# sag111/ContiniousEnvironment_Follower_Leader

Measured on AMD Instinct MI355X. Metric: env-steps/sec at 65,536 parallel envs; 1/2/4/8 MI355X scaling, higher is better.
Workload: dtype f64

## Files before the change

continiousenvironment_follower_leader_amd/_lib.py:

```python
import ctypes as C
import os
import subprocess

from . import abi

_PKG = os.path.dirname(os.path.abspath(__file__))
_ROOT = os.path.dirname(_PKG)
SO_PATH = os.path.join(_PKG, "libftl_hip.so")
SOURCES = [os.path.join(_PKG, "csrc", "ftl_abi.hip"), os.path.join(_PKG, "csrc", "ftl_device.hpp"),
           os.path.join(_PKG, "csrc", "ftl_frames_group.hpp"), os.path.join(_PKG, "csrc", "ftl_aux.hpp"), os.path.join(_PKG, "csrc", "ftl_gazebo.hpp"), os.path.join(_ROOT, "include", "ftl_gazebo.h"), os.path.join(_PKG, "csrc", "ftl_scenario.cpp"),
           os.path.join(_PKG, "csrc", "ftl_scenario_dev.hpp"),
           os.path.join(_PKG, "csrc", "ftl_crmath.hpp"),
           os.path.join(_PKG, "csrc", "ftl_render.hpp"),
           os.path.join(_PKG, "csrc", "ftl_snapshot.hpp"),
           os.path.join(_PKG, "csrc", "ftl_queue.hpp"),
           os.path.join(_PKG, "csrc", "ftl_sampler.hpp"),
           os.path.join(_ROOT, "include", "ftl.h")]
UNITS = [os.path.join(_PKG, "csrc", "ftl_abi.hip"), os.path.join(_PKG, "csrc", "ftl_scenario.cpp")]
HIPCC = os.environ.get("HIPCC", "/opt/rocm/bin/hipcc")
HIPCC_FLAGS = ["--offload-arch=gfx950", "-O3", "-ffp-contract=off", "-fPIC", "-shared", "-std=c++17"]

_LIB = None


def build(force=False, verbose=False):
    stale = (not os.path.exists(SO_PATH)) or any(os.path.getmtime(s) > os.path.getmtime(SO_PATH) for s in SOURCES)
    if force or stale:
        cmd = [HIPCC] + HIPCC_FLAGS + ["-pthread", "-o", SO_PATH] + UNITS
        if verbose:
            print(" ".join(cmd))
        subprocess.check_call(cmd, cwd=os.path.join(_PKG, "csrc"))
    return SO_PATH


class FtlError(RuntimeError):
    pass


def load():
    global _LIB
    if _LIB is not None:
        return _LIB
    so_path = os.environ.get("FTL_LIB", SO_PATH)
    if not os.path.exists(so_path):
        raise FtlError("libftl_hip.so is not built (run `python -c 'import __graft_entry__ as g; g.build()'`); "
                       "there is no CPU fallback")
    import torch
    lib = C.CDLL(so_path)
    vp, i32, u32 = C.c_void_p, C.c_int32, C.c_uint32
    lib.ftl_last_error.restype = C.c_char_p
    lib.ftl_create.argtypes = [C.POINTER(abi.Config), i32, i32, C.POINTER(vp)]
    lib.ftl_create.restype = C.c_int
    lib.ftl_destroy.argtypes = [vp]
    lib.ftl_destroy.restype = None
    lib.ftl_lasers_len.argtypes = [vp]
    lib.ftl_lasers_len.restype = i32
    lib.ftl_get_config.argtypes = [vp, C.POINTER(abi.Config)]
    lib.ftl_state_bytes.argtypes = [vp]
    lib.ftl_state_bytes.restype = C.c_size_t
    lib.ftl_bind_state.argtypes = [vp, vp, C.c_size_t]
    lib.ftl_state_field.argtypes = [vp, C.c_char_p, C.POINTER(C.c_size_t), C.POINTER(C.c_size_t), C.POINTER(i32), C.POINTER(C.c_size_t)]
    lib.ftl_load_scenarios.argtypes = [vp, C.POINTER(abi.Scenarios)]
    lib.ftl_set_reset_window.argtypes = [vp, i32, i32, i32]
    lib.ftl_tune.argtypes = [vp, i32, i32]
    lib.ftl_reset.argtypes = [vp, vp, vp, C.POINTER(abi.Outputs), vp]
    lib.ftl_step.argtypes = [vp, vp, C.POINTER(abi.Outputs), u32, vp]
    lib.ftl_step_encoded.argtypes = [vp, vp, i32, C.POINTER(abi.Outputs), u32, vp]
    lib.ftl_step_final.argtypes = [vp, vp, i32, C.POINTER(abi.Outputs), C.POINTER(abi.FinalOutputs), u32, vp]
    lib.ftl_kernel_timing.argtypes = [vp, i32]
    lib.ftl_kernel_times.argtypes = [vp, C.POINTER(C.c_double * 4), C.POINTER(i32)]
    lib.ftl_episode_metrics.argtypes = [vp, vp, vp, u32, vp]
    lib.ftl_episode_metrics.restype = C.c_int
    lib.ftl_generate_scenarios.argtypes = [C.POINTER(abi.Config), C.POINTER(abi.ScenParams), vp, i32, i32,
                                           C.POINTER(abi.Scenarios), vp]
    lib.ftl_generate_scenarios.restype = C.c_int
    lib.ftl_sizeof_scen_params.restype = C.c_size_t
    lib.ftl_generate_scenarios_device_workspace.argtypes = [C.POINTER(abi.Config), C.POINTER(abi.ScenParams), i32, C.POINTER(C.c_size_t)]
    lib.ftl_generate_scenarios_device_workspace.restype = C.c_int
    lib.ftl_generate_scenarios_device.argtypes = [C.POINTER(abi.Config), C.POINTER(abi.ScenParams), vp, i32, C.POINTER(abi.Scenarios), vp,
                                                  vp, C.c_size_t, vp]
    lib.ftl_generate_scenarios_device.restype = C.c_int
    lib.ftl_sizeof_render_params.restype = C.c_size_t
    lib.ftl_render_workspace.argtypes = [vp, i32, C.POINTER(C.c_size_t)]
    lib.ftl_render_workspace.restype = C.c_int
    lib.ftl_render.argtypes = [vp, vp, i32, C.POINTER(abi.RenderParams), vp, C.c_size_t, vp, vp]
    lib.ftl_render.restype = C.c_int
    lib.ftl_env_bytes.argtypes = [vp]
    lib.ftl_env_bytes.restype = C.c_size_t
    lib.ftl_env_layout_id.argtypes = [vp]
    lib.ftl_env_layout_id.restype = C.c_uint64
    lib.ftl_pack_envs.argtypes = [vp, vp, i32, vp, vp]
    lib.ftl_pack_envs.restype = C.c_int
    lib.ftl_unpack_envs.argtypes = [vp, vp, vp, i32, u32, vp]
    lib.ftl_unpack_envs.restype = C.c_int
    lib.ftl_sizeof_episode_record.restype = C.c_size_t
    lib.ftl_sizeof_episode_queue.restype = C.c_size_t
    lib.ftl_set_episode_queue.argtypes = [vp, C.POINTER(abi.EpisodeQueueC)]
    lib.ftl_set_episode_queue.restype = C.c_int
    lib.ftl_queue_start.argtypes = [vp, C.POINTER(abi.Outputs), vp]
    lib.ftl_queue_start.restype = C.c_int
    lib.ftl_sizeof_scenario_sampler.restype = C.c_size_t
    lib.ftl_set_scenario_sampler.argtypes = [vp, C.POINTER(abi.ScenarioSamplerC)]
    lib.ftl_set_scenario_sampler.restype = C.c_int
    lib.ftl_sampler_refresh.argtypes = [vp, vp]
    lib.ftl_sampler_refresh.restype = C.c_int
    lib.ftl_sampler_start.argtypes = [vp, C.POINTER(abi.Outputs), vp]
    lib.ftl_sampler_start.restype = C.c_int
    lib.ftl_gz_create.argtypes = [vp, i32, i32, C.POINTER(vp)]
    lib.ftl_gz_destroy.argtypes = [vp]
    lib.ftl_gz_destroy.restype = None
    lib.ftl_gz_state_bytes.argtypes = [vp]
    lib.ftl_gz_state_bytes.restype = C.c_size_t
    lib.ftl_gz_bind_state.argtypes = [vp, vp, C.c_size_t]
    lib.ftl_gz_lasers_len.argtypes = [vp]
    lib.ftl_gz_lasers_len.restype = i32
    lib.ftl_gz_reset.argtypes = [vp, vp, vp]
    lib.ftl_gz_step.argtypes = [vp, vp, vp, vp, vp, vp, vp, vp, vp]
    lib.ftl_gz_state_field.argtypes = [vp, C.c_char_p, C.POINTER(C.c_size_t), C.POINTER(C.c_size_t), C.POINTER(i32)]
    for n in ("ftl_sizeof_config", "ftl_sizeof_scenarios", "ftl_sizeof_outputs", "ftl_sizeof_final_outputs"):
        getattr(lib, n).restype = C.c_size_t
    _LIB = lib
    return lib


EXPORTS = ("ftl_create", "ftl_destroy", "ftl_lasers_len", "ftl_get_config", "ftl_state_bytes", "ftl_bind_state",
           "ftl_state_field", "ftl_load_scenarios", "ftl_set_reset_window", "ftl_tune", "ftl_reset", "ftl_step", "ftl_step_encoded", "ftl_step_final", "ftl_last_error", "ftl_generate_scenarios",
           "ftl_generate_scenarios_device_workspace", "ftl_generate_scenarios_device",
           "ftl_episode_metrics", "ftl_kernel_timing", "ftl_kernel_times",
           "ftl_sizeof_render_params", "ftl_render_workspace", "ftl_render",
           "ftl_env_bytes", "ftl_env_layout_id", "ftl_pack_envs", "ftl_unpack_envs",
           "ftl_sizeof_episode_record", "ftl_sizeof_episode_queue", "ftl_set_episode_queue", "ftl_queue_start",
           "ftl_sizeof_scenario_sampler", "ftl_set_scenario_sampler", "ftl_sampler_refresh", "ftl_sampler_start",
           "ftl_gz_create", "ftl_gz_destroy", "ftl_gz_state_bytes", "ftl_gz_bind_state", "ftl_gz_lasers_len", "ftl_gz_reset", "ftl_gz_step",
           "ftl_gz_state_field")


def check(rc, lib=None):
    if rc != 0:
        lib = lib or load()
        msg = lib.ftl_last_error().decode("utf-8", "replace")
        if rc == abi.FTL_E_INVALID:
            raise ValueError(msg)
        if rc == abi.FTL_E_UNSUPPORTED:
            raise NotImplementedError(msg)
        raise FtlError("ftl error %d: %s" % (rc, msg))
```

continiousenvironment_follower_leader_amd/abi.py:

```python
import ctypes as C

FTL_ABI_VERSION = 4
FTL_MAX_BEARS = 6
FTL_MAX_LASERS = 4
FTL_MAX_AUX = 8
AUX_LIDAR, AUX_TRACK_VECTOR, AUX_TRACK_RADAR = 1, 2, 3
FTL_MAX_REGIME = 16
FTL_OBS_NUM = 10

FTL_OK = 0
FTL_E_INVALID, FTL_E_UNSUPPORTED, FTL_E_DEVICE, FTL_E_STATE = -1, -2, -3, -4

MISSION = ("in_progress", "fail", "success", "finished_by_time")
AGENT = ("moving", "crash", "low_reward", "too_far_from_leader", "finished")
LEADER = ("moving", "crash", "finished")

FTL_ERR_TRAJ_OVERFLOW, FTL_ERR_CORR_OVERFLOW, FTL_ERR_EMPTY_CORRIDOR, FTL_ERR_TRACKER_SEED, FTL_ERR_HIST1_OVERFLOW = 1, 2, 4, 8, 16
FTL_ERR_LIDAR_OVERFLOW = 32
FTL_ERR_BAD_ACTION = 64
FTL_ERR_BAD_STREAM = 128
FTL_ACTION_BOX2, FTL_ACTION_DISCRETE, FTL_ACTION_TURN = 0, 1, 2
FTL_STEP_AUTO_RESET = 1
FTL_STEP_NEXT_RESET = 4
FTL_STEP_QUEUE_RESET = 8
FTL_STEP_SAMPLE_RESET = 16
FTL_EPISODE_DONE_AT_RESET = 1
FTL_N_SCEN_STATS = 10
(SS_EPISODES, SS_FRAMES_SUM, SS_SUCCESS, SS_CRASH, SS_LOW_REWARD, SS_TOO_FAR, SS_TIMEOUT, SS_RETURN_Q16, SS_DONE_AT_RESET,
 SS_LAST_CALL) = range(10)
SS_NAMES = ("episodes", "frames_sum", "success", "crash", "low_reward", "too_far", "timeout", "return_q16", "done_at_reset", "last_call")
FTL_N_METRICS = 8
FTL_METRICS_CLEAR = 1
(M_EPISODES, M_RETURN_SUM, M_FRAMES_SUM, M_SUCCESS, M_CRASH, M_LOW_REWARD, M_TOO_FAR, M_TIMEOUT) = range(8)

(EI_SCEN, EI_TARGET_ID, EI_LEADER_FINISHED, EI_DONE, EI_CRASH, EI_IN_BOX, EI_ON_TRACE, EI_TOO_CLOSE,
 EI_STEP_COUNT, EI_FINISH_TIMER, EI_TRAJ_LEN, EI_TRK_COUNTER, EI_CORR_LO, EI_CORR_HI, EI_SEED_END,
 EI_SNAP_COUNT, EI_DYN_INDEX0, EI_DYN_INDEX1, EI_DYN_INDEX2, EI_DYN_INDEX3, EI_DYN_INDEX4, EI_DYN_INDEX5, EI_ERROR, EI_EPISODES,
 EI_GREEN_COUNT, EI_GREEN_LEN, EI_SCAN_OK, EI_SNAP_HEAD, EI_HINT, EI_GREEN_TINY, EI_RESETS, EI_ACC_CONSUMED,
 EI_HINT_X, EI_HINT_Y, EI_CLR_GREEN, EI_CLR_ALL, EI_FPS, EI_HW0_LO, EI_HW0_HI, EI_HIST1_LEN, EI_ERROR_STICKY, EI_STREAM, EI_COUNT) = range(43)
FTL_ENV_SLOT_STATS, FTL_ENV_OWN_STREAM = 1, 2
ED_ACC_PENALTY, ED_OVERALL_REWARD, ED_SPARE0, ED_SPARE1, ED_BEAR_POINTS = range(5)
ED_GREEN_W = ED_BEAR_POINTS + 2 * FTL_MAX_BEARS
ED_CUR_MULT, ED_CUR_ACC, ED_CUM_SPEED = ED_GREEN_W + 1, ED_GREEN_W + 2, ED_GREEN_W + 3
ED_COUNT = ED_CUM_SPEED + 1
RD_DIRECTION, RD_SPEED, RD_ROT_SPEED, RD_DES_SPEED, RD_DES_ROT_SPEED, RD_COUNT = range(6)
RI_X, RI_Y, RI_W, RI_H, RI_ROT_DIR, RI_DES_ROT_DIR, RI_SPARE0, RI_SPARE1, RI_COUNT = range(9)


def rand_frames(rng_seed, env_id, resets, step_count, lo, hi):
    v = lo + int(uniform01(rng_seed, env_id, resets, step_count | (1 << 40)) * (hi - lo))
    return v if v < hi else hi - 1


def rand_range(rng_seed, env_id, resets, frame, bear, k, start, stop):
    n = (stop - start + 9) // 10
    v = int(uniform01(rng_seed, env_id, resets, frame | (1 << 41) | (bear << 44) | (k << 48)) * n)
    return start + 10 * (v if v < n else n - 1)


class RobotParams(C.Structure):
    _fields_ = [("min_speed", C.c_double), ("max_speed", C.c_double), ("max_rotation_speed", C.c_double),
                ("max_speed_change", C.c_double), ("max_rotation_speed_change", C.c_double),
                ("img_w", C.c_int32), ("img_h", C.c_int32), ("_pad", C.c_int32 * 2)]


class LaserCfg(C.Structure):
    _fields_ = [("count", C.c_int32), ("react_corridor", C.c_int32), ("react_green", C.c_int32),
                ("react_obstacles", C.c_int32), ("history", C.c_int32), ("after_tracker", C.c_int32),
                ("out_offset", C.c_int32), ("pad_sectors", C.c_int32), ("lenient", C.c_int32), ("in_policy_obs", C.c_int32),
                ("length", C.c_double), ("angle_offset", C.c_double),
                ("explicit_angles", C.c_int32), ("compas", C.c_int32), ("ray_angles", C.c_double * 8)]


class AuxCfg(C.Structure):
    _fields_ = [("kind", C.c_int32), ("after_tracker", C.c_int32), ("out_offset", C.c_int32), ("out_len", C.c_int32),
                ("n_angles", C.c_int32), ("points_number", C.c_int32), ("return_all_points", C.c_int32),
                ("return_only_distances", C.c_int32), ("range_px", C.c_double), ("in_range_px", C.c_double),
                ("angle_step", C.c_double), ("border_angle", C.c_int32), ("seq_len", C.c_int32),
                ("detectable", C.c_int32), ("radar_sectors", C.c_int32)]


class Config(C.Structure):
    _fields_ = [("abi_version", C.c_int32), ("width", C.c_int32), ("height", C.c_int32),
                ("frames_per_step", C.c_int32), ("max_steps", C.c_int32), ("warm_start", C.c_int32),
                ("trajectory_saving_period", C.c_int32), ("n_static", C.c_int32), ("n_bears", C.c_int32),
                ("move_bear_v4", C.c_int32), ("ignore_follower_collisions", C.c_int32),
                ("aggregate_reward", C.c_int32), ("has_low_reward", C.c_int32),
                ("has_max_distance_coef", C.c_int32), ("has_tracker", C.c_int32),
                ("tracker_saving_period", C.c_int32), ("tracker_start_behind", C.c_int32),
                ("n_lasers", C.c_int32), ("traj_cap", C.c_int32), ("corr_cap", C.c_int32),
                ("route_cap", C.c_int32), ("init_traj_cap", C.c_int32), ("hist1_cap", C.c_int32), ("trk1_eat_close_points", C.c_int32),
                ("low_reward", C.c_double), ("max_distance_coef", C.c_double),
                ("min_distance", C.c_double), ("max_distance", C.c_double), ("max_dev", C.c_double),
                ("leader_pos_epsilon", C.c_double), ("corridor_length", C.c_double),
                ("corridor_width", C.c_double),
                ("reward_in_box", C.c_double), ("reward_on_track", C.c_double), ("reward_in_dev", C.c_double),
                ("not_on_track_penalty", C.c_double), ("crash_penalty", C.c_double),
                ("too_close_penalty", C.c_double), ("leader_movement_reward", C.c_double),
                ("leader", RobotParams), ("follower", RobotParams), ("bear", RobotParams),
                ("lasers", LaserCfg * FTL_MAX_LASERS),
                ("n_speed_regime", C.c_int32), ("n_acc_regime", C.c_int32),
                ("speed_key", C.c_int32 * FTL_MAX_REGIME), ("speed_is_range", C.c_int32 * FTL_MAX_REGIME),
                ("acc_key", C.c_int32 * FTL_MAX_REGIME), ("env_id_base", C.c_int32),
                ("rand_fps_lo", C.c_int32), ("rand_fps_hi", C.c_int32), ("_pad1", C.c_int32),
                ("speed_lo", C.c_double * FTL_MAX_REGIME), ("speed_hi", C.c_double * FTL_MAX_REGIME),
                ("acc_val", C.c_double * FTL_MAX_REGIME), ("rng_seed", C.c_uint64),
                ("trk1_eat_radius", C.c_double), ("n_aux", C.c_int32), ("_pad2", C.c_int32), ("aux", AuxCfg * FTL_MAX_AUX)]


_M64 = (1 << 64) - 1


def mix64(x):
    x &= _M64
    x ^= x >> 30; x = (x * 0xBF58476D1CE4E5B9) & _M64
    x ^= x >> 27; x = (x * 0x94D049BB133111EB) & _M64
    x ^= x >> 31
    return x


def uniform01(rng_seed, env_id, resets, frame):
    key = mix64(rng_seed + 0x9E3779B97F4A7C15 * (env_id + 1)) ^ mix64(0xD1B54A32D192ED03 * (resets + 1))
    return (mix64(key + 0x9E3779B97F4A7C15 * (frame + 1)) >> 11) * (1.0 / 9007199254740992.0)


def mulhi64(a, b):
    return ((a & _M64) * (b & _M64)) >> 64


def sample_scenario(rng_seed, stream_id, resets, cdf, base=0):
    key = mix64(rng_seed + 0x9E3779B97F4A7C15 * (stream_id + 1)) ^ mix64(0xD1B54A32D192ED03 * (resets + 1))
    x = mix64(key + 0x9E3779B97F4A7C15 * ((1 << 42) + 1))
    count = len(cdf)
    total = int(cdf[count - 1])
    if total == 0:
        return base + mulhi64(x, count)
    r = mulhi64(x, total)
    lo, hi = 0, count - 1
    while lo < hi:
        mid = lo + (hi - lo) // 2
        if int(cdf[mid]) <= r:
            lo = mid + 1
        else:
            hi = mid
    return base + lo


class Scenarios(C.Structure):
    _fields_ = [("n_scenarios", C.c_int32), ("_pad", C.c_int32),
                ("static_rects", C.c_void_p), ("robot_pos", C.c_void_p), ("robot_dir", C.c_void_p),
                ("robot_rect", C.c_void_p), ("route", C.c_void_p), ("route_len", C.c_void_p),
                ("init_traj", C.c_void_p), ("init_traj_len", C.c_void_p)]


class ScenParams(C.Structure):
    _fields_ = [("width", C.c_int32), ("height", C.c_int32), ("step_grid", C.c_int32), ("obstacle_number", C.c_int32),
                ("add_obstacles", C.c_int32), ("add_bear", C.c_int32), ("bear_number", C.c_int32), ("bear_behind", C.c_int32),
                ("multiple_end_points", C.c_int32), ("path_finding_iterations", C.c_int32),
                ("bridge_gap", C.c_int32), ("bridge_width", C.c_int32),
                ("trajectory_saving_period", C.c_int32), ("planner", C.c_int32),
                ("min_distance", C.c_double), ("max_distance", C.c_double),
                ("leader_pos_epsilon", C.c_double), ("leader_margin", C.c_double),
                ("leader_w", C.c_double), ("leader_h", C.c_double), ("leader_max_speed", C.c_double),
                ("fixed_route", C.c_void_p), ("fixed_route_len", C.c_int32), ("_pad", C.c_int32)]


SCEN_FOUND, SCEN_DONE_AT_RESET, SCEN_ROUTE_OVERFLOW, SCEN_TRAJ_OVERFLOW, SCEN_REF_RAISES = 1, 2, 4, 8, 16
SCEN_GEN_LIMIT = 32


class Outputs(C.Structure):
    _fields_ = [("obs_num", C.c_void_p), ("lasers", C.c_void_p), ("target", C.c_void_p),
                ("reward", C.c_void_p), ("done", C.c_void_p), ("status", C.c_void_p), ("policy_obs", C.c_void_p)]

FTL_TUNE_COSCHEDULED_ENVS, FTL_TUNE_REGROUP_EVERY, FTL_TUNE_TWO_STREAMS = 0, 1, 2


class FinalOutputs(C.Structure):
    _fields_ = [("obs_num", C.c_void_p), ("lasers", C.c_void_p), ("target", C.c_void_p), ("policy_obs", C.c_void_p),
                ("ended", C.c_void_p), ("restarted", C.c_void_p)]


class EpisodeRecord(C.Structure):
    _fields_ = [("state", C.c_int32), ("scenario", C.c_int32), ("env", C.c_int32), ("frames", C.c_int32), ("calls", C.c_int32),
                ("status", C.c_int32 * 3), ("errors", C.c_uint32), ("flags", C.c_uint32), ("ret", C.c_double), ("stream", C.c_int64)]


RECORD_DTYPE = [("state", "<i4"), ("scenario", "<i4"), ("env", "<i4"), ("frames", "<i4"), ("calls", "<i4"), ("status", "<i4", (3,)),
                ("errors", "<u4"), ("flags", "<u4"), ("ret", "<f8"), ("stream", "<i8")]


class EpisodeQueueC(C.Structure):
    _fields_ = [("scenario", C.c_void_p), ("stream", C.c_void_p), ("stream_base", C.c_int64), ("n", C.c_int32), ("_pad", C.c_int32),
                ("head", C.c_void_p), ("records", C.c_void_p), ("ticket", C.c_void_p)]


class ScenarioSamplerC(C.Structure):
    _fields_ = [("weight", C.c_void_p), ("cdf", C.c_void_p), ("base", C.c_int32), ("count", C.c_int32), ("table", C.c_void_p)]


RENDER_PATH, RENDER_BOX, RENDER_OBJECTS, RENDER_RECTS, RENDER_SENSORS, RENDER_TARGET = 1, 2, 4, 8, 16, 32
RENDER_ALL = 63


class RenderParams(C.Structure):
    _fields_ = [("width", C.c_int32), ("height", C.c_int32), ("scale", C.c_float), ("origin_x", C.c_float), ("origin_y", C.c_float),
                ("layers", C.c_uint32), ("_pad", C.c_int32)]
```

continiousenvironment_follower_leader_amd/csrc/ftl_abi.hip:

```cpp
#include <hip/hip_runtime.h>

#include <cstdio>
#include <cstring>
#include <new>
#include <string>
#include <vector>

#include <cstdlib>
#include <cmath>

#include "ftl_device.hpp"
#include "ftl_frames_group.hpp"
#include "ftl_aux.hpp"

namespace {

thread_local std::string g_err;

int fail(int code, const std::string& msg) { g_err = msg; return code; }

struct Field { const char* name; size_t offset, per_env; int dtype; size_t stride; };
constexpr int FTL_N_FIELDS = 15;

}

struct FtlQueueState;
struct FtlSamplerState;

struct ftl_handle {
    FtlDevParams P;
    FtlDevParams* dP;
    bool dirty;
    int device;
    size_t state_bytes;
    Field fields[FTL_N_FIELDS];
    void* mt_mem;
    bool timing;
    std::vector<hipEvent_t> tev;
    size_t tev_used;
    bool bound, have_scen;
    bool regroup;
    void* rg_mem;
    int* rg_tot;
    unsigned rg_parity, rg_launches, rg_every;
    bool rg_env, rg_every_env, split_env;
    int G;
    int co_envs, cus;
    bool g_env;
    int rg_slots, rg_epw;
    hipStream_t side; hipEvent_t ev_fork, ev_join; bool split;
    int win_base, win_count, win_stride;
    size_t lds_pad;
    float* last_lasers;
    FtlQueueState* queue;
    FtlSamplerState* sampler;
};

static void ftl_queue_destroy(ftl_handle* h);
static int ftl_queue_attached(const ftl_handle* h);
static int ftl_queue_finish_step(ftl_handle* h, const FtlCall& step, const ftl_outputs* out, const ftl_final_outputs* fin, void* stream);
static void ftl_sampler_destroy(ftl_handle* h);
static int ftl_sampler_attached(const ftl_handle* h);
static int ftl_sampler_check_window(const ftl_handle* h);
static int ftl_sampler_finish_step(ftl_handle* h, const FtlCall& step, const ftl_outputs* out, const ftl_final_outputs* fin, void* stream);

namespace {

size_t align_up(size_t v, size_t a) { return (v + a - 1) / a * a; }

int validate(const ftl_config& c, std::string& why) {
    char buf[256];
#define REQ(cond, ...) do { if (!(cond)) { snprintf(buf, sizeof buf, __VA_ARGS__); why = buf; return FTL_E_INVALID; } } while (0)
    REQ(c.abi_version == FTL_ABI_VERSION, "abi_version %d != %d", c.abi_version, FTL_ABI_VERSION);
    REQ(c.width > 0 && c.height > 0, "bad field size");
    REQ(c.frames_per_step > 0, "frames_per_step must be positive");
    REQ(c.rand_fps_hi == 0 || (c.rand_fps_lo > 0 && c.rand_fps_lo < c.rand_fps_hi), "random_frames_per_step must be (low, high) with 0 < low < high");
    REQ(c.trajectory_saving_period > 0, "trajectory_saving_period must be positive");
    REQ(c.n_static >= 0 && c.n_static <= 4096, "n_static out of range");
    REQ(c.n_bears >= 0 && c.n_bears <= FTL_MAX_BEARS, "n_bears out of range (0..%d)", FTL_MAX_BEARS);
    REQ(c.n_lasers >= 0 && c.n_lasers <= FTL_MAX_LASERS, "n_lasers out of range");
    REQ(c.n_lasers == 0 || c.has_tracker, "ray sensors need the tracker (classes.py:280 would raise NameError)");
    REQ(c.traj_cap >= 8 && c.corr_cap >= 8 && c.corr_cap <= 512 && c.route_cap >= 2 && c.init_traj_cap >= 1, "bad capacities");
    REQ((c.corr_cap & (c.corr_cap - 1)) == 0, "corr_cap must be a power of two (the tracker rings are indexed with a mask)");
    REQ(c.init_traj_cap <= c.traj_cap, "init_traj_cap > traj_cap");
    REQ(c.traj_cap % FTL_TRAJ_BLOCK == 0, "traj_cap must be a multiple of FTL_TRAJ_BLOCK");
    if (c.has_tracker == 2) {
        REQ(c.tracker_saving_period > 0, "tracker saving_period must be positive");
        REQ(c.corridor_length > 0 && c.corridor_width > 0, "corridor_length / corridor_width must be positive");
    }
    REQ(c.n_speed_regime <= FTL_MAX_REGIME && c.n_acc_regime <= FTL_MAX_REGIME, "too many regime entries");
    REQ(c.has_tracker >= 0 && c.has_tracker <= 2, "has_tracker must be 0, 1 (v1) or 2 (v2)");
    if (c.has_tracker == 1) REQ(c.tracker_saving_period > 0 && c.hist1_cap >= 8 && c.corridor_width > 0, "bad v1 tracker parameters");
    REQ(c.n_aux >= 0 && c.n_aux <= FTL_MAX_AUX, "n_aux out of range");
    for (int j = 0; j < c.n_aux; j++) {
        const ftl_aux_cfg& a = c.aux[j];
        REQ(a.kind >= FTL_AUX_LIDAR && a.kind <= FTL_AUX_TRACK_RADAR, "aux %d: unknown sensor kind", j);
        if (a.kind == FTL_AUX_LIDAR) {
            REQ(a.n_angles > 0 && a.n_angles <= 512 && a.points_number > 0 && a.range_px > 0, "aux %d: bad lidar parameters", j);
            REQ(a.points_number <= 1024 && a.n_angles * a.points_number < 65536, "aux %d: lidar with more than 1024 points per ray or 65535 (ray, point) pairs", j);
        }
        else {
            REQ(c.has_tracker != 0, "aux %d: a leader-track detector needs a tracker (classes.py:272 would raise NameError)", j);
            REQ(a.seq_len > 0 && a.detectable >= 0 && a.detectable <= (a.kind == FTL_AUX_TRACK_RADAR ? 2 : 1), "aux %d: bad detector parameters", j);
            if (a.kind == FTL_AUX_TRACK_RADAR) REQ(a.radar_sectors > 0 && a.radar_sectors <= 4096, "aux %d: bad radar_sectors_number", j);
        }
    }
    for (int k = 0; k < c.n_lasers; k++) {
        const ftl_laser_cfg& l = c.lasers[k];
        REQ(l.count > 0 && l.count <= 1024, "laser %d: bad lasers_count", k);
        REQ(l.history > 0 && l.history <= FTL_HMAX, "laser %d: max_prev_obs must be in 1..%d", k, FTL_HMAX);
        REQ(l.react_obstacles >= 0 && l.react_obstacles <= 3, "laser %d: bad react_to_obstacles", k);
        REQ(l.length > 0, "laser %d: bad laser_length", k);
    }
#undef REQ
    return FTL_OK;
}

}

extern "C" {

const char* ftl_last_error(void) { return g_err.c_str(); }

size_t ftl_sizeof_config(void) { return sizeof(ftl_config); }
size_t ftl_sizeof_scenarios(void) { return sizeof(ftl_scenarios); }
size_t ftl_sizeof_outputs(void) { return sizeof(ftl_outputs); }
size_t ftl_sizeof_scen_params(void) { return sizeof(ftl_scen_params); }
size_t ftl_sizeof_final_outputs(void) { return sizeof(ftl_final_outputs); }

static int set_lanes(ftl_handle* h) {
    FtlDevParams& P = h->P;
    const ftl_config* cfg = &P.cfg;
    if (!h->g_env) h->G = (P.R > 4 || h->co_envs <= h->cus * 4 * 8) ? 8 : 4;
    if (P.R > 4) h->G = 8;
    const int epw = FTL_WAVE / h->G;
    h->rg_epw = epw;
    const int f_max = cfg->rand_fps_hi > 0 ? cfg->rand_fps_hi - 1 : cfg->frames_per_step;
    size_t o = align_up((size_t)epw * cfg->n_static * 16 + (size_t)epw * 4 + 32, 16);
    P.fr_rec_stride = (int)align_up((size_t)f_max, 16);
    P.fr_rec_off = (int)o; o += (size_t)P.fr_rec_stride * epw;
    P.fr_pend_off = (int)o; o += (size_t)epw * (P.fr_defer ? f_max - 1 : 1) * 16;
    P.fr_env_off = (int)o; o += (size_t)epw * 4 + 16 + (size_t)epw * 16;
    P.fr_lds = (int)o;
    h->dirty = true;
    return o > 64 * 1024 ? 1 : 0;
}

int ftl_create(const ftl_config* cfg, int32_t n_envs, int32_t device, ftl_handle** out) {
    if (!cfg || !out) return fail(FTL_E_INVALID, "null argument");
    if (n_envs <= 0) return fail(FTL_E_INVALID, "n_envs must be positive");
    if (device < 0) return fail(FTL_E_INVALID, "device < 0: this library has no CPU path");
    std::string why;
    int rc = validate(*cfg, why);
    if (rc) return fail(rc, why);
    ftl_handle* h = new (std::nothrow) ftl_handle();
    if (!h) return fail(FTL_E_DEVICE, "out of host memory");
    memset(&h->P, 0, sizeof h->P);
    h->P.cfg = *cfg;
    for (int k = 0; k < FTL_MAX_LASERS; k++) h->P.cfg.lasers[k].after_tracker = cfg->lasers[k].after_tracker ? 1 : 0;
    h->device = device;
    h->bound = false; h->have_scen = false; h->dP = nullptr; h->dirty = true;
    h->rg_mem = nullptr; h->rg_tot = nullptr; h->rg_parity = 0; h->rg_launches = 0; h->mt_mem = nullptr; h->timing = false; h->tev_used = 0;
    h->side = nullptr; h->ev_fork = nullptr; h->ev_join = nullptr; h->last_lasers = nullptr; h->queue = nullptr; h->sampler = nullptr;
    {
        const char* sp = getenv("FTL_SPLIT");
        h->split = n_envs >= 8192 && (sp ? sp[0] == '1' : cfg->rand_fps_hi > 0) && cfg->has_tracker != 1;
        h->split_env = sp != nullptr;
    }
    {
        const char* off = getenv("FTL_NO_REGROUP");
        const char* ev = getenv("FTL_REGROUP_EVERY");
        h->rg_every = (ev && atoi(ev) > 0) ? (unsigned)atoi(ev) : 4u;
        int cus = 256;
        (void)hipDeviceGetAttribute(&cus, hipDeviceAttributeMultiprocessorCount, device);
        const char* g8 = getenv("FTL_DEBUG_G8");
        h->g_env = g8 != nullptr; h->cus = cus; h->co_envs = n_envs;
        h->G = (2 + cfg->n_bears > 4 || (g8 ? g8[0] == '1' : n_envs <= cus * 4 * 8)) ? 8 : 4;
        const int epw_f = FTL_WAVE / h->G;
        const bool beyond_one_round = (n_envs + epw_f - 1) / epw_f > cus * 4 * FTL_FRAMESG_WPE;
        h->regroup = (off ? off[0] != '1' : (beyond_one_round || cfg->rand_fps_hi > 0)) && (n_envs + FTL_RG_BLOCK - 1) / FTL_RG_BLOCK <= 512;
        h->rg_env = off != nullptr; h->rg_every_env = ev && atoi(ev) > 0; h->rg_slots = cus * 4 * FTL_FRAMESG_WPE; h->rg_epw = epw_f;
    }
    FtlDevParams& P = h->P;
    P.n_envs = n_envs;
    P.R = 2 + cfg->n_bears;
    int off = 0, hmax = 1, rays = 0;
    auto width_of = [](const ftl_laser_cfg& l) { return l.count * (l.compas ? 5 : (l.pad_sectors ? 4 : 1)); };
    for (int k = 0; k < cfg->n_lasers; k++) {
        P.cfg.lasers[k].out_offset = off;
        off += cfg->lasers[k].history * width_of(cfg->lasers[k]);
        hmax = cfg->lasers[k].history > hmax ? cfg->lasers[k].history : hmax;
        rays += cfg->lasers[k].count;
    }
    for (int j = 0; j < cfg->n_aux; j++) {
        ftl_aux_cfg& a = P.cfg.aux[j];
        a.out_len = a.kind == FTL_AUX_LIDAR ? (a.return_all_points ? 1 + a.n_angles * a.points_number * (a.return_only_distances ? 1 : 2) : a.n_angles * (a.return_only_distances ? 1 : 2))
                  : a.kind == FTL_AUX_TRACK_VECTOR ? 2 * a.seq_len : a.radar_sectors;
        a.out_offset = off; off += a.out_len;
    }
    P.lasers_len = off; P.total_rays = rays; P.hmax = hmax;
    {
        const double deg2rad = 3.141592653589793 / 180.0;
        bool miss_ok = true;
        const double span = (double)(cfg->width > cfg->height ? cfg->width : cfg->height);
        const double margin = 1e-11 * (span > 2048.0 ? span / 2048.0 : 1.0);
        for (int k = 0; k < cfg->n_lasers; k++) {
            const ftl_laser_cfg& l = cfg->lasers[k];
            miss_ok = miss_ok && (float)(l.length - margin) == (float)l.length && (float)(l.length + margin) == (float)l.length;
        }
        P.miss_const = miss_ok ? 1 : 0;
        int rb[2] = {0, 0};
        for (int k = 0; k < cfg->n_lasers; k++) {
            const ftl_laser_cfg& l = cfg->lasers[k];
            FtlRaySensor& rs = P.ray_sens[k];
            const int which = l.after_tracker ? 1 : 0, ro = l.react_obstacles;
            rs.count = l.count; rs.rbase = rb[which];
            rs.reach2 = ((float)l.length + 2.0f) * ((float)l.length + 2.0f);
            rs.inv_step = (float)l.count * 0.15915494309189535f; rs.inv_count = 1.0f / (float)l.count;
            rs.off_u = (float)(l.angle_offset * deg2rad) * rs.inv_step;
            rs.slack = 0.022f + 0.01f * (float)l.count * 0.15915494f;
            rs.flags = ((ro == 1 || ro == 2) ? 1u : 0u) | ((ro == 1 || ro == 3) ? 2u : 0u) | (l.react_corridor ? 4u : 0u) | (l.react_green ? 8u : 0u)
                     | (l.explicit_angles ? 16u : 0u) | (which ? 32u : 0u) | (l.compas ? 64u : 0u);
            if (!l.compas) rb[which] += l.count;
        }
        P.inv_nrect_dyn = (65536u + (unsigned)(P.R - 1) - 1u) / (unsigned)(P.R - 1);
        int g = 0;
        for (int which = 0; which < 2; which++) {
            P.pass_base[which] = g; P.pass_lmax[which] = 0.0f;
            for (int k = 0; k < cfg->n_lasers; k++) {
                const ftl_laser_cfg& l = cfg->lasers[k];
                if ((l.after_tracker ? 1 : 0) != which || l.compas) continue;
                P.pass_lmax[which] = fmaxf(P.pass_lmax[which], (float)l.length);
                for (int i = 0; i < l.count && g < FTL_MAX_RAYS; i++, g++) {
                    const double a = l.explicit_angles ? l.ray_angles[i & 7] : l.angle_offset + i * (360.0 / (double)l.count);
                    P.ray_dir[g].c = cos(a * deg2rad); P.ray_dir[g].s = sin(a * deg2rad); P.ray_dir[g].len = l.length;
                }
            }
            P.pass_rays[which] = g - P.pass_base[which];
        }
    }
    if (rays > 1023) { delete h; return fail(FTL_E_INVALID, "more than 1023 rays per env (the candidate list of the ray kernel packs a ray index into 10 bits)"); }
    if (hmax * (P.R - 1) > FTL_WAVE) { delete h; return fail(FTL_E_INVALID, "max_prev_obs x (1 + bears) exceeds one wavefront of snapshot rects"); }
    {
        int w = 0, hcommon = 0;
        for (int k = 0; k < cfg->n_lasers; k++) {
            P.pol_off[k] = -1;
            if (!cfg->lasers[k].in_policy_obs) continue;
            P.pol_off[k] = w; w += width_of(cfg->lasers[k]);
            if (hcommon == 0) hcommon = cfg->lasers[k].history;
            else if (cfg->lasers[k].history != hcommon) hcommon = -1;
        }
        P.pol_width = w; P.pol_h = hcommon;
    }
    const size_t n = (size_t)n_envs;
    struct { const char* name; size_t per_env; int dtype; size_t esz; bool rec; } spec[FTL_N_FIELDS] = {
        {"rb_pos", (size_t)P.R * 2, 1, 4, true}, {"rb_dbl", (size_t)P.R * FTL_RD_COUNT, 2, 8, true}, {"rb_int", (size_t)P.R * FTL_RI_COUNT, 0, 4, true},
        {"env_int", FTL_EI_COUNT, 0, 4, true}, {"env_dbl", FTL_ED_COUNT, 2, 8, true}, {"traj", (size_t)cfg->traj_cap * 2, 1, 4, false},
        {"hist", (size_t)cfg->corr_cap * 2, 2, 8, false}, {"corr", (size_t)cfg->corr_cap * 4, 2, 8, false},
        {"snap_rects", (size_t)hmax * (P.R - 1) * 4, 0, 4, true}, {"snap_win", (size_t)hmax * 4, 0, 4, true},
        {"traj_bb", (size_t)(cfg->traj_cap / FTL_TRAJ_BLOCK) * 4, 1, 4, false}, {"ep_stats", FTL_N_METRICS, 2, 8, false},
        {"hist1", (size_t)(cfg->has_tracker == 1 ? cfg->hist1_cap : 0) * 2, 1, 4, false}, {"fol_cs", 2, 2, 8, true},
        {"corr32", (size_t)cfg->corr_cap * 4, 1, 4, false}};
    static const int rec_order[8] = {3 , 13 , 0 , 1 , 9 , 8 , 4 , 2 };
    size_t ro = 0;
    for (int k = 0; k < 8; k++) {
        const int i = rec_order[k];
        ro = align_up(ro, 16);
        h->fields[i] = Field{spec[i].name, ro, spec[i].per_env, spec[i].dtype, 0};
        ro += spec[i].per_env * spec[i].esz;
    }
    const size_t rec_stride = align_up(ro, 128);
    P.rec_stride = (int32_t)rec_stride;
    for (int k = 0; k < 8; k++) h->fields[rec_order[k]].stride = rec_stride;
    size_t cur = rec_stride * n;
    for (int i = 0; i < FTL_N_FIELDS; i++) {
        if (spec[i].rec) continue;
        cur = align_up(cur, 256);
        h->fields[i] = Field{spec[i].name, cur, spec[i].per_env, spec[i].dtype, spec[i].per_env * spec[i].esz};
        cur += spec[i].per_env * spec[i].esz * n;
    }
    h->state_bytes = align_up(cur, 256);
    {
        const size_t rects = (size_t)cfg->n_static + hmax + (size_t)hmax * (P.R - 2 > 0 ? P.R - 2 : 0) + 1;
        P.corr_lds_cap = cfg->corr_cap < 128 ? cfg->corr_cap : 128;
        if (const char* lc = getenv("FTL_DEBUG_CORR_LDS_CAP")) { int v = atoi(lc); if (v >= 2 && v <= cfg->corr_cap && (v & (v - 1)) == 0) P.corr_lds_cap = v; }
        P.lds_rays = (int)((size_t)P.corr_lds_cap * 16 + rects * 20 + (size_t)2 * P.corr_lds_cap * 4 + (size_t)2 * hmax * 20 + 64
                           + (size_t)rays * 16 + (size_t)rays * (hmax <= 5 ? 5 : FTL_HMAX) * 4       + (size_t)rays * 4
                           + rects * 8 + 32
                           + (size_t)FTL_PAIR_CAP * 2 + 16);
    }
    {
        const int f_max = cfg->rand_fps_hi > 0 ? cfg->rand_fps_hi - 1 : cfg->frames_per_step;
        const char* dv = getenv("FTL_DEFER");
        P.fr_defer = (cfg->rand_fps_hi == 0 && f_max >= 2 && f_max <= 16 && cfg->traj_cap <= 65535 && !(dv && dv[0] == '0')) ? 1 : 0;
        if (cfg->traj_cap > 65535 || f_max > 4095) { delete h; return fail(FTL_E_INVALID, "traj_cap above 65535 or more than 4095 frames per step"); }
        if (set_lanes(h)) { delete h; return fail(FTL_E_INVALID, "the frame kernel needs more than 64 KiB of LDS per wavefront (static rects x frames per step)"); }
    }
    auto debug_pad = [](const char* name) { const char* v = getenv(name); const int p = v ? atoi(v) : 0; return p < 0 ? 0 : (p > 48 * 1024 ? 48 * 1024 : p); };
    P.lds_rays += debug_pad("FTL_DEBUG_LDS_PAD_RAYS");
    h->lds_pad = (size_t)debug_pad("FTL_DEBUG_LDS_PAD");
    if (getenv("FTL_DEBUG_PRINT_LDS")) fprintf(stderr, "ftl: ray kernel LDS %d B per env\n", P.lds_rays);
    if (P.lds_rays > 64 * 1024) { delete h; return fail(FTL_E_INVALID, "config needs more than 64 KiB of LDS per env"); }
    if (ftl_aux_lds_bytes(*cfg) > 64 * 1024) { delete h; return fail(FTL_E_INVALID, "the compas / lidar / radar sensors of this config need more than 64 KiB of LDS per env"); }
    *out = h;
    return FTL_OK;
}

void ftl_destroy(ftl_handle* h) {
    if (!h) return;
    if (h->dP || h->rg_mem || h->side || h->mt_mem) (void)hipSetDevice(h->device);
    ftl_queue_destroy(h);
    ftl_sampler_destroy(h);
    if (h->dP) (void)hipFree(h->dP);
    if (h->mt_mem) (void)hipFree(h->mt_mem);
    for (hipEvent_t ev : h->tev) (void)hipEventDestroy(ev);
    if (h->rg_mem) (void)hipFree(h->rg_mem);
    if (h->side) { (void)hipStreamSynchronize(h->side); (void)hipStreamDestroy(h->side); }
    if (h->ev_fork) (void)hipEventDestroy(h->ev_fork);
    if (h->ev_join) (void)hipEventDestroy(h->ev_join);
    delete h;
}

int32_t ftl_lasers_len(const ftl_handle* h) { return h ? h->P.lasers_len : 0; }

int ftl_get_config(const ftl_handle* h, ftl_config* out) {
    if (!h || !out) return fail(FTL_E_INVALID, "null argument");
    *out = h->P.cfg;
    return FTL_OK;
}

size_t ftl_state_bytes(const ftl_handle* h) { return h ? h->state_bytes : 0; }

int ftl_state_field(const ftl_handle* h, const char* name, size_t* offset, size_t* per_env, int32_t* dtype, size_t* stride) {
    if (!h || !name) return fail(FTL_E_INVALID, "null argument");
    for (int i = 0; i < FTL_N_FIELDS; i++)
        if (!strcmp(h->fields[i].name, name)) {
            if (offset) *offset = h->fields[i].offset;
            if (per_env) *per_env = h->fields[i].per_env;
            if (dtype) *dtype = h->fields[i].dtype;
            if (stride) *stride = h->fields[i].stride;
            return FTL_OK;
        }
    return fail(FTL_E_INVALID, std::string("unknown state field ") + name);
}

int ftl_bind_state(ftl_handle* h, void* dev_state, size_t bytes) {
    if (!h || !dev_state) return fail(FTL_E_INVALID, "null argument");
    if (bytes < h->state_bytes) return fail(FTL_E_INVALID, "state buffer too small");
    if (((uintptr_t)dev_state) & 255) return fail(FTL_E_INVALID, "state buffer must be 256-byte aligned");
    unsigned char* b = (unsigned char*)dev_state;
    FtlDevParams& P = h->P;
    P.rb_pos = (float*)(b + h->fields[0].offset); P.rb_dbl = (double*)(b + h->fields[1].offset); P.rb_int = (int32_t*)(b + h->fields[2].offset);
    P.env_int = (int32_t*)(b + h->fields[3].offset); P.env_dbl = (double*)(b + h->fields[4].offset); P.traj = (float*)(b + h->fields[5].offset);
    P.hist = (double*)(b + h->fields[6].offset); P.corr = (double*)(b + h->fields[7].offset);
    P.snap_rects = (int32_t*)(b + h->fields[8].offset); P.snap_win = (int32_t*)(b + h->fields[9].offset);
    P.traj_bb = (float*)(b + h->fields[10].offset); P.ep_stats = (double*)(b + h->fields[11].offset);
    P.hist1 = (float*)(b + h->fields[12].offset); P.fol_cs = (double*)(b + h->fields[13].offset); P.corr32 = (float*)(b + h->fields[14].offset);
    h->bound = true; h->dirty = true;
    return FTL_OK;
}

int ftl_load_scenarios(ftl_handle* h, const ftl_scenarios* pool) {
    if (!h || !pool) return fail(FTL_E_INVALID, "null argument");
    if (pool->n_scenarios <= 0) return fail(FTL_E_INVALID, "empty scenario pool");
    if (!pool->robot_pos || !pool->robot_dir || !pool->robot_rect || !pool->route || !pool->route_len ||
        !pool->init_traj || !pool->init_traj_len || (h->P.cfg.n_static > 0 && !pool->static_rects))
        return fail(FTL_E_INVALID, "scenario pool has null arrays");
    h->P.scen = *pool;
    h->have_scen = true; h->dirty = true;
    h->win_base = 0; h->win_count = pool->n_scenarios; h->win_stride = h->P.n_envs % pool->n_scenarios;
    return FTL_OK;
}

int ftl_set_reset_window(ftl_handle* h, int32_t base, int32_t count, int32_t stride) {
    if (!h) return fail(FTL_E_INVALID, "null argument");
    if (!h->have_scen) return fail(FTL_E_STATE, "ftl_load_scenarios has not been called");
    if (base < 0 || count <= 0 || base + count > h->P.scen.n_scenarios) return fail(FTL_E_INVALID, "reset window outside the scenario pool");
    h->win_base = base; h->win_count = count; h->win_stride = (stride > 0 ? stride : h->P.n_envs) % count;
    return FTL_OK;
}

int ftl_tune(ftl_handle* h, int32_t what, int32_t value) {
    if (!h) return fail(FTL_E_INVALID, "null argument");
    switch (what) {
    case FTL_TUNE_COSCHEDULED_ENVS:
        if (value < h->P.n_envs) return fail(FTL_E_INVALID, "co-scheduled envs below this handle's own");
        h->co_envs = value;
        if (set_lanes(h)) return fail(FTL_E_INVALID, "the frame kernel needs more than 64 KiB of LDS per wavefront (static rects x frames per step)");
        if (!h->rg_env)
            h->regroup = ((value + h->rg_epw - 1) / h->rg_epw > h->rg_slots || h->P.cfg.rand_fps_hi > 0) && (h->P.n_envs + FTL_RG_BLOCK - 1) / FTL_RG_BLOCK <= 512;
        return FTL_OK;
    case FTL_TUNE_REGROUP_EVERY:
        if (value < 1) return fail(FTL_E_INVALID, "regroup interval below 1");
        if (!h->rg_every_env) h->rg_every = (unsigned)value;
        return FTL_OK;
    case FTL_TUNE_TWO_STREAMS:
        if (!h->split_env) h->split = value != 0 && h->P.n_envs >= 8192 && h->P.cfg.has_tracker != 1;
        return FTL_OK;
    }
    return fail(FTL_E_INVALID, "unknown tuning key");
}

static int sync_params(ftl_handle* h) {
    hipError_t e;
    if (!h->dP) {
        e = hipMalloc((void**)&h->dP, sizeof(FtlDevParams));
        if (e != hipSuccess) return fail(FTL_E_DEVICE, std::string("hipMalloc(params): ") + hipGetErrorString(e));
        h->dirty = true;
    }
    if (h->dirty) {
        e = hipMemcpy(h->dP, &h->P, sizeof(FtlDevParams), hipMemcpyHostToDevice);
        if (e != hipSuccess) return fail(FTL_E_DEVICE, std::string("hipMemcpy(params): ") + hipGetErrorString(e));
        h->dirty = false;
    }
    return FTL_OK;
}

static int launch(ftl_handle* h, const FtlCall& call, void* stream) {
    hipError_t e = hipSetDevice(h->device);
    if (e != hipSuccess) return fail(FTL_E_DEVICE, std::string("hipSetDevice: ") + hipGetErrorString(e));
    if (h->regroup && !h->rg_mem) {
        const size_t n = (size_t)h->P.n_envs, nb = (n + FTL_RG_BLOCK - 1) / FTL_RG_BLOCK;
        const size_t o_bh = align_up(n * 4, 256), o_rank = o_bh + align_up(nb * FTL_NKEYS * 4, 256), o_keys = o_rank + align_up(n * 2, 256), o_tot = o_keys + align_up(n, 256);
        e = hipMalloc(&h->rg_mem, o_tot + 2 * FTL_NKEYS * sizeof(int));
        if (e != hipSuccess) return fail(FTL_E_DEVICE, std::string("hipMalloc(regroup): ") + hipGetErrorString(e));
        char* b = (char*)h->rg_mem;
        h->P.perm = (int32_t*)b; h->P.bh = (int32_t*)(b + o_bh); h->P.rank = (uint16_t*)(b + o_rank); h->P.keys = (uint8_t*)(b + o_keys);
        h->rg_tot = (int*)(b + o_tot); h->rg_parity = 0;
        e = hipMemsetAsync(h->rg_tot, 0, 2 * FTL_NKEYS * sizeof(int), (hipStream_t)stream);
        if (e != hipSuccess) return fail(FTL_E_DEVICE, std::string("hipMemsetAsync(regroup): ") + hipGetErrorString(e));
        hipLaunchKernelGGL(ftl::ftl_perm_identity_kernel, dim3((unsigned)((n + 255) / 256)), dim3(256), 0, (hipStream_t)stream, h->P.perm, (int)n);
        h->dirty = true;
    }
    { int rc = sync_params(h); if (rc) return rc; }
    if (h->split && !h->side) {
        if (hipStreamCreateWithFlags(&h->side, hipStreamNonBlocking) != hipSuccess ||
            hipEventCreateWithFlags(&h->ev_fork, hipEventDisableTiming) != hipSuccess ||
            hipEventCreateWithFlags(&h->ev_join, hipEventDisableTiming) != hipSuccess)
            return fail(FTL_E_DEVICE, "cannot create the side stream / events");
    }
    hipEvent_t* tev = nullptr;
    if (h->timing && !h->split && call.mode == 0 && h->tev_used + 5 <= 5 * 512) {
        while (h->tev.size() < h->tev_used + 5) { hipEvent_t ev; if (hipEventCreate(&ev) != hipSuccess) return fail(FTL_E_DEVICE, "hipEventCreate"); h->tev.push_back(ev); }
        tev = h->tev.data() + h->tev_used; h->tev_used += 5;
    }
    const bool xr = (call.flags & (FTL_STEP_NEXT_RESET | FTL_CALL_DEFER_RESET | FTL_CALL_FINISH)) != 0 || call.ended || call.restarted;
    auto launch_range = [&](int part, int parts, hipStream_t s) {
        const int epw0 = FTL_WAVE / h->G;
        const int n_groups = (h->P.n_envs + epw0 - 1) / epw0;
        const int my_groups = (n_groups - part + parts - 1) / parts;
        FtlCall c2 = call; c2.part = part; c2.parts = parts; c2.epw = epw0;
        const int count = my_groups * epw0;
        const bool reg = h->P.cfg.n_speed_regime >= 0 || h->P.cfg.n_acc_regime >= 0 || h->P.cfg.rand_fps_hi > 0;
        const int epw = FTL_WAVE / h->G;
        size_t lds = (size_t)h->P.fr_lds + h->lds_pad;
        const dim3 grid((count + epw - 1) / epw), block(FTL_WAVE);
        if (tev) (void)hipEventRecord(tev[0], s);
        if (xr) {
            if (h->G == 4) {
                if (reg) hipLaunchKernelGGL((ftl_frames_group_kernel<4, true, true>), grid, block, lds, s, h->dP, c2);
                else hipLaunchKernelGGL((ftl_frames_group_kernel<4, false, true>), grid, block, lds, s, h->dP, c2);
            } else {
                if (reg) hipLaunchKernelGGL((ftl_frames_group_kernel<8, true, true>), grid, block, lds, s, h->dP, c2);
                else hipLaunchKernelGGL((ftl_frames_group_kernel<8, false, true>), grid, block, lds, s, h->dP, c2);
            }
        } else if (h->G == 4) {
            if (reg) hipLaunchKernelGGL((ftl_frames_group_kernel<4, true>), grid, block, lds, s, h->dP, c2);
            else hipLaunchKernelGGL((ftl_frames_group_kernel<4, false>), grid, block, lds, s, h->dP, c2);
        } else {
            if (reg) hipLaunchKernelGGL((ftl_frames_group_kernel<8, true>), grid, block, lds, s, h->dP, c2);
            else hipLaunchKernelGGL((ftl_frames_group_kernel<8, false>), grid, block, lds, s, h->dP, c2);
        }
        if (h->P.cfg.has_tracker == 1 && part == 0)
            hipLaunchKernelGGL(ftl::ftl_tracker1_kernel, dim3((unsigned)((h->P.n_envs + 255) / 256)), dim3(256), 0, s, h->dP, c2);
        if (tev) (void)hipEventRecord(tev[1], s);
        if (h->P.cfg.n_lasers > 0) {
            bool expl = false;
            for (int k = 0; k < h->P.cfg.n_lasers; k++) expl = expl || h->P.cfg.lasers[k].explicit_angles != 0 || h->P.cfg.lasers[k].pad_sectors != 0 || h->P.cfg.lasers[k].compas != 0;
            const dim3 rgrid(count);
#define FTL_LAUNCH_RAYS(HM_, EXPL_, SPLIT_) do { \
                if (capped) hipLaunchKernelGGL((ftl_rays_kernel<HM_, EXPL_, SPLIT_, true>), rgrid, block, h->P.lds_rays, s, h->dP, c2); \
                else hipLaunchKernelGGL((ftl_rays_kernel<HM_, EXPL_, SPLIT_, false>), rgrid, block, h->P.lds_rays, s, h->dP, c2); } while (0)
            const bool capped = h->P.corr_lds_cap < h->P.cfg.corr_cap;
            if (parts > 1) {
                if (!expl && h->P.hmax > 5 && h->P.hmax <= 10) FTL_LAUNCH_RAYS(10, false, true);
                else if (h->P.hmax <= 5) FTL_LAUNCH_RAYS(5, true, true);
                else FTL_LAUNCH_RAYS(FTL_HMAX, true, true);
            } else if (expl) {
                if (h->P.hmax <= 5) FTL_LAUNCH_RAYS(5, true, false);
                else FTL_LAUNCH_RAYS(FTL_HMAX, true, false);
            } else if (h->P.hmax <= 5) FTL_LAUNCH_RAYS(5, false, false);
            else if (h->P.hmax <= 8) FTL_LAUNCH_RAYS(8, false, false);
            else if (h->P.hmax <= 10) FTL_LAUNCH_RAYS(10, false, false);
            else FTL_LAUNCH_RAYS(FTL_HMAX, false, false);
#undef FTL_LAUNCH_RAYS
        }
        if (tev) (void)hipEventRecord(tev[2], s);
    };
    if (h->split) {
        (void)hipEventRecord(h->ev_fork, (hipStream_t)stream);
        (void)hipStreamWaitEvent(h->side, h->ev_fork, 0);
        launch_range(0, 2, (hipStream_t)stream);
        launch_range(1, 2, h->side);
        (void)hipEventRecord(h->ev_join, h->side);
        (void)hipStreamWaitEvent((hipStream_t)stream, h->ev_join, 0);
    } else launch_range(0, 1, (hipStream_t)stream);
    {
        bool aux = h->P.cfg.n_aux > 0;
        for (int k = 0; k < h->P.cfg.n_lasers; k++) aux = aux || h->P.cfg.lasers[k].compas != 0;
        if (aux) hipLaunchKernelGGL(ftl_aux_kernel, dim3((unsigned)h->P.n_envs), dim3(FTL_WAVE), ftl_aux_lds_bytes(h->P.cfg), (hipStream_t)stream, h->dP, call);
    }
    if (tev) (void)hipEventRecord(tev[3], (hipStream_t)stream);
    if (h->regroup && !(call.flags & FTL_CALL_FINISH) && (h->P.cfg.rand_fps_hi > 0 || call.mode == 1 || (h->rg_launches++ % h->rg_every) == 0)) {
        const unsigned nb = (unsigned)((h->P.n_envs + FTL_RG_BLOCK - 1) / FTL_RG_BLOCK);
        int* tot = h->rg_tot + (h->rg_parity & 1u) * FTL_NKEYS, *tot_next = h->rg_tot + ((h->rg_parity + 1u) & 1u) * FTL_NKEYS;
        h->rg_parity++;
        hipLaunchKernelGGL(ftl::ftl_regroup_count_kernel, dim3(nb), dim3(FTL_RG_BLOCK), 0, (hipStream_t)stream, h->dP, tot);
        hipLaunchKernelGGL(ftl::ftl_regroup_scatter_kernel, dim3(nb), dim3(FTL_RG_BLOCK), 0, (hipStream_t)stream, h->dP, (const int*)tot, tot_next);
    }
    if (tev) (void)hipEventRecord(tev[4], (hipStream_t)stream);
    e = hipGetLastError();
    if (e != hipSuccess) return fail(FTL_E_DEVICE, std::string("kernel launch: ") + hipGetErrorString(e));
    return FTL_OK;
}

static int check_out(const ftl_handle* h, const ftl_outputs* out) {
    if (!out || !out->obs_num || !out->target || !out->reward || !out->done || !out->status || (h->P.lasers_len > 0 && !out->lasers))
        return fail(FTL_E_INVALID, "output arrays missing");
    return FTL_OK;
}

int ftl_reset(ftl_handle* h, const int32_t* scen_idx, const uint8_t* mask, const ftl_outputs* out, void* stream) {
    if (!h || !scen_idx) return fail(FTL_E_INVALID, "null argument");
    if (!h->bound) return fail(FTL_E_STATE, "ftl_bind_state has not been called");
    if (!h->have_scen) return fail(FTL_E_STATE, "ftl_load_scenarios has not been called");
    int rc = check_out(h, out);
    if (rc) return rc;
    if (out->policy_obs && h->P.pol_h <= 0) return fail(FTL_E_INVALID, "policy_obs needs the same max_prev_obs on every ray sensor");
    FtlCall call; call.mode = 1; call.scen_idx = scen_idx; call.mask = mask; call.out = *out; call.action = nullptr; call.flags = 0; call.action_kind = FTL_ACTION_BOX2; call.win_base = h->win_base; call.win_count = h->win_count; call.win_stride = h->win_stride;
    call.ended = nullptr; call.restarted = nullptr;
    h->last_lasers = h->P.lasers_len > 0 ? out->lasers : nullptr;
    return launch(h, call, stream);
}

int ftl_step(ftl_handle* h, const double* action, const ftl_outputs* out, uint32_t flags, void* stream) {
    return ftl_step_encoded(h, action, FTL_ACTION_BOX2, out, flags, stream);
}

int ftl_step_encoded(ftl_handle* h, const void* action, int32_t encoding, const ftl_outputs* out, uint32_t flags, void* stream) {
    return ftl_step_final(h, action, encoding, out, nullptr, flags, stream);
}

int ftl_step_final(ftl_handle* h, const void* action, int32_t encoding, const ftl_outputs* out, const ftl_final_outputs* fin,
                   uint32_t flags, void* stream) {
    if (!h || !action) return fail(FTL_E_INVALID, "null argument");
    flags &= FTL_STEP_AUTO_RESET | FTL_STEP_NEXT_RESET | FTL_STEP_QUEUE_RESET | FTL_STEP_SAMPLE_RESET;
    if ((flags & FTL_STEP_AUTO_RESET) && (flags & FTL_STEP_NEXT_RESET)) return fail(FTL_E_INVALID, "FTL_STEP_AUTO_RESET and FTL_STEP_NEXT_RESET exclude each other");
    const bool queue = (flags & FTL_STEP_QUEUE_RESET) != 0;
    if (queue && flags != FTL_STEP_QUEUE_RESET) return fail(FTL_E_INVALID, "FTL_STEP_QUEUE_RESET excludes the other reset flags");
    const bool sample = (flags & FTL_STEP_SAMPLE_RESET) != 0;
    if (sample && flags != FTL_STEP_SAMPLE_RESET) return fail(FTL_E_INVALID, "FTL_STEP_SAMPLE_RESET excludes the other reset flags");
    if (encoding < FTL_ACTION_BOX2 || encoding > FTL_ACTION_TURN) return fail(FTL_E_INVALID, "unknown action encoding");
    if (sample && !ftl_sampler_attached(h)) return fail(FTL_E_STATE, "FTL_STEP_SAMPLE_RESET without a scenario sampler (ftl_set_scenario_sampler)");
    if (queue && !ftl_queue_attached(h)) return fail(FTL_E_STATE, "FTL_STEP_QUEUE_RESET without an episode queue (ftl_set_episode_queue)");
    if (!h->bound) return fail(FTL_E_STATE, "ftl_bind_state has not been called");
    if (!h->have_scen) return fail(FTL_E_STATE, "ftl_load_scenarios has not been called");
    int rc = check_out(h, out);
    if (rc) return rc;
    if (out->policy_obs && h->P.pol_h <= 0) return fail(FTL_E_INVALID, "policy_obs needs the same max_prev_obs on every ray sensor");
    const bool same_step = fin && (flags & (FTL_STEP_AUTO_RESET | FTL_STEP_QUEUE_RESET | FTL_STEP_SAMPLE_RESET));
    if (fin && (!fin->ended || !fin->restarted)) return fail(FTL_E_INVALID, "ftl_final_outputs: ended / restarted missing");
    if (same_step && (!fin->obs_num || !fin->target || (h->P.lasers_len > 0 && !fin->lasers)))
        return fail(FTL_E_INVALID, "ftl_final_outputs: obs_num / lasers / target missing (needed under FTL_STEP_AUTO_RESET / FTL_STEP_QUEUE_RESET / FTL_STEP_SAMPLE_RESET)");
    if (same_step && fin->policy_obs && !out->policy_obs) return fail(FTL_E_INVALID, "ftl_final_outputs.policy_obs needs ftl_outputs.policy_obs");
    FtlCall call; call.mode = 0; call.action = (const double*)action; call.action_kind = encoding; call.out = *out; call.flags = flags; call.scen_idx = nullptr; call.mask = nullptr; call.win_base = h->win_base; call.win_count = h->win_count; call.win_stride = h->win_stride;
    call.ended = fin ? fin->ended : nullptr; call.restarted = fin ? fin->restarted : nullptr;
    h->last_lasers = h->P.lasers_len > 0 ? out->lasers : nullptr;
    if (queue) {
        call.flags = 0; call.ended = nullptr; call.restarted = nullptr;
        rc = launch(h, call, stream);
        return rc ? rc : ftl_queue_finish_step(h, call, out, fin, stream);
    }
    if (sample) {
        rc = ftl_sampler_check_window(h);
        if (rc) return rc;
        call.flags = 0; call.ended = nullptr; call.restarted = nullptr;
        rc = launch(h, call, stream);
        return rc ? rc : ftl_sampler_finish_step(h, call, out, fin, stream);
    }
    if (!same_step) return launch(h, call, stream);
    call.flags = (flags & ~(uint32_t)FTL_STEP_AUTO_RESET) | FTL_CALL_DEFER_RESET;
    rc = launch(h, call, stream);
    if (rc) return rc;
    const int n = h->P.n_envs, epb = FTL_FC_THREADS;
    const int pol_len = (fin->policy_obs && out->policy_obs) ? h->P.pol_h * h->P.pol_width : 0;
    hipLaunchKernelGGL(ftl::ftl_final_copy_kernel, dim3((unsigned)((n + epb - 1) / epb)), dim3(FTL_FC_THREADS), 0, (hipStream_t)stream,
                       *out, *fin, n, h->P.lasers_len, pol_len);
    FtlCall rcall = call;
    rcall.mode = 1; rcall.flags = FTL_CALL_FINISH; rcall.mask = fin->ended; rcall.action = nullptr; rcall.ended = nullptr; rcall.restarted = nullptr;
    return launch(h, rcall, stream);
}

int ftl_kernel_timing(ftl_handle* h, int32_t enable) {
    if (!h) return fail(FTL_E_INVALID, "null argument");
    if (enable && h->split) return fail(FTL_E_UNSUPPORTED, "per-kernel timing is not available in the two-stream mode");
    h->timing = enable != 0; h->tev_used = 0;
    return FTL_OK;
}

int ftl_kernel_times(ftl_handle* h, double* ms, int32_t* n_steps) {
    if (!h || !ms || !n_steps) return fail(FTL_E_INVALID, "null argument");
    if (h->split) return fail(FTL_E_UNSUPPORTED, "per-kernel timing is not available in the two-stream mode");
    ms[0] = ms[1] = ms[2] = ms[3] = 0.0; *n_steps = 0;
    if (h->tev_used == 0) return FTL_OK;
    (void)hipSetDevice(h->device);
    hipError_t e = hipEventSynchronize(h->tev[h->tev_used - 1]);
    if (e != hipSuccess) return fail(FTL_E_DEVICE, std::string("hipEventSynchronize: ") + hipGetErrorString(e));
    for (size_t i = 0; i + 5 <= h->tev_used; i += 5) {
        for (int k = 0; k < 4; k++) {
            float t = 0.0f;
            e = hipEventElapsedTime(&t, h->tev[i + k], h->tev[i + k + 1]);
            if (e != hipSuccess) return fail(FTL_E_DEVICE, std::string("hipEventElapsedTime: ") + hipGetErrorString(e));
            ms[k] += (double)t;
        }
        *n_steps += 1;
    }
    h->tev_used = 0;
    return FTL_OK;
}

int ftl_episode_metrics(ftl_handle* h, double* dev_metrics, int32_t* dev_errors, uint32_t flags, void* stream) {
    if (!h || !dev_metrics) return fail(FTL_E_INVALID, "null argument");
    if (!h->bound) return fail(FTL_E_STATE, "ftl_bind_state has not been called");
    hipError_t e = hipSetDevice(h->device);
    if (e != hipSuccess) return fail(FTL_E_DEVICE, std::string("hipSetDevice: ") + hipGetErrorString(e));
    const int nb = (h->P.n_envs + FTL_MT_BLOCK - 1) / FTL_MT_BLOCK;
    const size_t o_err = align_up((size_t)nb * FTL_N_METRICS * sizeof(double), 256);
    if (!h->mt_mem) {
        e = hipMalloc(&h->mt_mem, o_err + (size_t)nb * 2 * sizeof(int));
        if (e != hipSuccess) return fail(FTL_E_DEVICE, std::string("hipMalloc(metrics): ") + hipGetErrorString(e));
    }
    { int rc = sync_params(h); if (rc) return rc; }
    double* part = (double*)h->mt_mem; int* epart = (int*)((char*)h->mt_mem + o_err);
    hipLaunchKernelGGL(ftl::ftl_metrics_partial_kernel, dim3((unsigned)nb), dim3(FTL_MT_THREADS), 0, (hipStream_t)stream, h->dP, part, epart, (flags & FTL_METRICS_CLEAR) ? 1 : 0);
    hipLaunchKernelGGL(ftl::ftl_metrics_final_kernel, dim3(1), dim3(64), 0, (hipStream_t)stream, (const double*)part, (const int*)epart, nb, dev_metrics, dev_errors);
    e = hipGetLastError();
    if (e != hipSuccess) return fail(FTL_E_DEVICE, std::string("kernel launch: ") + hipGetErrorString(e));
    return FTL_OK;
}

}

#include "ftl_gazebo.hpp"
#include "ftl_scenario_dev.hpp"
#include "ftl_render.hpp"
#include "ftl_snapshot.hpp"
#include "ftl_queue.hpp"
#include "ftl_sampler.hpp"

#ifdef FTL_WAVE_TIMES
extern "C" int ftl_debug_wave_timeline(unsigned long long* times, unsigned int* info) {
    hipDeviceSynchronize();
    return hipMemcpyFromSymbol(times, HIP_SYMBOL(ftl::g_wt), sizeof(unsigned long long) * 2 * 8192) != hipSuccess ||
           hipMemcpyFromSymbol(info, HIP_SYMBOL(ftl::g_wi), sizeof(unsigned int) * 8192) != hipSuccess;
}
#endif
#ifdef FTL_PROFILE_PATHS
extern "C" int ftl_debug_heavy(unsigned long long* out, int clear) {
    hipDeviceSynchronize();
    if (hipMemcpyFromSymbol(out, HIP_SYMBOL(ftl::g_cyc_heavy), sizeof(unsigned long long) * 17) != hipSuccess) return 1;
    if (clear) { unsigned long long z[17] = {0}; if (hipMemcpyToSymbol(HIP_SYMBOL(ftl::g_cyc_heavy), z, sizeof(z)) != hipSuccess) return 1; }
    return 0;
}
extern "C" int ftl_debug_wave_times(unsigned long long* out) {
    hipDeviceSynchronize();
    return hipMemcpyFromSymbol(out, HIP_SYMBOL(ftl::g_wave_t), sizeof(unsigned long long) * 2 * 8192) != hipSuccess;
}
extern "C" int ftl_debug_whist(unsigned int* out, int clear) {
    hipDeviceSynchronize();
    if (hipMemcpyFromSymbol(out, HIP_SYMBOL(ftl::g_whist), sizeof(unsigned int) * 128) != hipSuccess) return 1;
    if (clear) { unsigned int z[128] = {0}; if (hipMemcpyToSymbol(HIP_SYMBOL(ftl::g_whist), z, sizeof(z)) != hipSuccess) return 1; }
    return 0;
}
extern "C" int ftl_debug_prof(unsigned long long* out, int clear) {
    hipDeviceSynchronize();
    if (hipMemcpyFromSymbol(out, HIP_SYMBOL(ftl::g_prof), sizeof(unsigned long long) * 16) != hipSuccess) return 1;
    if (hipMemcpyFromSymbol(out + 16, HIP_SYMBOL(ftl::g_cyc), sizeof(unsigned long long) * 16) != hipSuccess) return 1;
#ifdef FTL_PROFILE_RAYS
    if (hipMemcpyFromSymbol(out + 32, HIP_SYMBOL(g_rcyc), sizeof(unsigned long long) * 16) != hipSuccess) return 1;
    if (clear) { unsigned long long z[16] = {0}; if (hipMemcpyToSymbol(HIP_SYMBOL(g_rcyc), z, sizeof(z)) != hipSuccess) return 1; }
#endif
    if (clear) { unsigned long long z[16] = {0}; if (hipMemcpyToSymbol(HIP_SYMBOL(ftl::g_prof), z, sizeof(z)) != hipSuccess) return 1;
                 if (hipMemcpyToSymbol(HIP_SYMBOL(ftl::g_cyc), z, sizeof(z)) != hipSuccess) return 1; }
    return 0;
}
#endif
```

continiousenvironment_follower_leader_amd/csrc/ftl_device.hpp:

```cpp
#pragma once
#include <hip/hip_runtime.h>
#include <stddef.h>
#include <stdint.h>

#include "../../include/ftl.h"

#define FTL_WAVE 64
#define FTL_HMAX 12
#define FTL_MAX_RAYS 1024
#ifndef FTL_WIDE_ARC
#define FTL_WIDE_ARC 3
#endif
#define FTL_PAIR_CAP (64 * FTL_WIDE_ARC)
#ifndef FTL_RAYS_WPE
#define FTL_RAYS_WPE 6
#endif

struct FtlRaySensor {
    int32_t count, rbase;
    float reach2;
    float inv_step, inv_count;
    float off_u;
    float slack;
    uint32_t flags;
};
struct alignas(16) FtlRayDir { double c, s, len, _pad; };
struct FtlDevParams {
    ftl_config cfg;
    int32_t n_envs, R, lasers_len, total_rays, hmax, lds_rays;
    int32_t pass_rays[2], pass_base[2];
    float pass_lmax[2];
    int32_t _pad_pass[2];
    int32_t fr_rec_off, fr_rec_stride, fr_pend_off, fr_env_off, fr_defer, fr_lds;
    int32_t corr_lds_cap;
    int32_t pol_off[FTL_MAX_LASERS], pol_width, pol_h;
    float* rb_pos; double* rb_dbl; int32_t* rb_int; int32_t* env_int; double* env_dbl;
    int32_t rec_stride, _pad_rec;
    float* traj; double* hist; double* corr; int32_t* snap_rects; int32_t* snap_win;
    float* traj_bb;
    double* ep_stats;
    float* corr32;
    float* hist1;
    double* fol_cs;
    FtlRayDir ray_dir[FTL_MAX_RAYS];
    FtlRaySensor ray_sens[FTL_MAX_LASERS];
    uint32_t inv_nrect_dyn;
    int32_t miss_const;
    int32_t* perm; uint8_t* keys; uint16_t* rank; int32_t* bh;
    ftl_scenarios scen;
};
static_assert(sizeof(FtlRayDir) == 32 && offsetof(FtlDevParams, ray_dir) % 32 == 0, "ray_dir: 16-byte loads of its records must be aligned, and a record must not straddle a cache line (the device copy is 256-byte aligned)");
struct FtlCall {
    const double* action; const int32_t* scen_idx; const uint8_t* mask;
    ftl_outputs out;
    uint32_t flags; int32_t mode;
    int32_t action_kind;
    int32_t win_base, win_count, win_stride;
    int32_t part, parts, epw;
    uint8_t* ended; uint8_t* restarted;
};
#define FTL_CALL_DEFER_RESET (1u << 30)
#define FTL_CALL_FINISH (1u << 29)
#define FTL_CALL_QUEUE (1u << 28)

template <typename T>
__device__ __forceinline__ T* rec_field(T* f0, const FtlDevParams& P, size_t env) {
    return reinterpret_cast<T*>(reinterpret_cast<char*>(f0) + env * (size_t)P.rec_stride);
}

namespace ftl {

static constexpr double kDeg2Rad = 3.141592653589793 / 180.0;
static constexpr double kRad2Deg = 180.0 / 3.141592653589793;

__device__ __forceinline__ void sincos_bounded(double x, double& s, double& c) {
    const double invpio2 = 6.36619772367581382433e-01;
    const double pio2_1 = 1.57079632673412561417e+00;
    const double pio2_2 = 6.07710050630396597660e-11, pio2_2t = 2.02226624879595063154e-21;
    double fn = rint(x * invpio2);
    int n = (int)fn;
    double t = x - fn * pio2_1;
    double w = fn * pio2_2;
    double r = t - w;
    w = fn * pio2_2t - ((t - r) - w);
    double y0 = r - w;
    double y1 = (r - y0) - w;
    const double S1 = -1.66666666666666324348e-01, S2 = 8.33333333332248946124e-03, S3 = -1.98412698298579493134e-04,
                 S4 = 2.75573137070700676789e-06, S5 = -2.50507602534068634195e-08, S6 = 1.58969099521155010221e-10;
    const double C1 = 4.16666666666666019037e-02, C2 = -1.38888888888741095749e-03, C3 = 2.48015872894767294178e-05,
                 C4 = -2.75573143513906633035e-07, C5 = 2.08757232129817482790e-09, C6 = -1.13596475577881948265e-11;
    double z = y0 * y0;
    double v = z * y0;
    double rs = S2 + z * (S3 + z * (S4 + z * (S5 + z * S6)));
    double ks = y0 - ((z * (0.5 * y1 - v * rs) - y1) - v * S1);
    double ww = z * z;
    double rc = z * (C1 + z * (C2 + z * C3)) + (ww * ww) * (C4 + z * (C5 + z * C6));
    double hz = 0.5 * z;
    double wc = 1.0 - hz;
    double kc = wc + (((1.0 - wc) - hz) + (z * rc - y0 * y1));
    int q = n & 3;
    double sv = (q & 1) ? kc : ks;
    double cv = (q & 1) ? ks : kc;
    s = (q & 2) ? -sv : sv;
    c = ((q + 1) & 2) ? -cv : cv;
}

__device__ __forceinline__ double euclid_f32(float ax, float ay, float bx, float by) {
    float dx = ax - bx, dy = ay - by;
    return (double)(float)sqrt((double)dx * (double)dx + (double)dy * (double)dy);
}
__device__ __forceinline__ double euclid_f64(double ax, double ay, double bx, double by) {
    double dx = ax - bx, dy = ay - by;
    return sqrt(dx * dx + dy * dy);
}
__device__ __forceinline__ bool euclid_f32_le(float ax, float ay, float bx, float by, double thr) {
    float dx = ax - bx, dy = ay - by;
    double x = (double)dx * (double)dx + (double)dy * (double)dy, t2 = thr * thr;
    if (x < t2 * (1.0 - 1e-6)) return true;
    if (x > t2 * (1.0 + 1e-6)) return false;
    return (double)(float)sqrt(x) <= thr;
}
__device__ __forceinline__ bool euclid_f64_lt(double ax, double ay, double bx, double by, double thr) {
    double dx = ax - bx, dy = ay - by;
    double x = dx * dx + dy * dy, t2 = thr * thr;
    if (x < t2 * (1.0 - 1e-12)) return true;
    if (x > t2 * (1.0 + 1e-12)) return false;
    return sqrt(x) < thr;
}
__device__ __forceinline__ double angle_correction(double a) {
    if (a >= 360.0) return a - 360.0;
    if (a < 0.0) return 360.0 + a;
    return a;
}
__device__ __forceinline__ double angle_to_point(double cx, double cy, double tx, double ty) {
    double rx = tx - cx, ry = ty - cy, res;
    if (rx > 0.0) res = atan(ry / rx) * kRad2Deg;
    else if (rx < 0.0) res = atan(ry / rx) * kRad2Deg + 180.0;
    else res = 0.0;
    return angle_correction(res);
}
__device__ __forceinline__ void rotate_size(int w, int h, double angle_deg, int& nw, int& nh) {
    double a = (double)(float)angle_deg;
    double q = rint(a / 90.0);
    if (q * 90.0 == a) {
        long long qi = (long long)(a / 90.0);
        if (qi & 1) { nw = h; nh = w; } else { nw = w; nh = h; }
        return;
    }
    double r = a * .01745329251994329, s, c;
    sincos_bounded(r, s, c);
    double cx = c * w, cy = c * h, sx = s * w, sy = s * h;
    double mx = fmax(fmax(fmax(fabs(cx + sy), fabs(cx - sy)), fabs(-cx + sy)), fabs(-cx - sy));
    double my = fmax(fmax(fmax(fabs(sx + cy), fabs(sx - cy)), fabs(-sx + cy)), fabs(-sx - cy));
    nw = (int)mx; nh = (int)my;
}

struct Robot {
    float px, py;
    double direction, speed, rot_speed, des_speed, des_rot_speed;
    int rot_dir, des_rot_dir;
    int rx, ry, rw, rh;
    double tgt_x, tgt_y;
    int dyn_index;
};
struct Limits { double min_speed, max_speed, max_rot, max_dv, max_drot; int img_w, img_h; };

__device__ __forceinline__ Limits lane_limits(const ftl_config& c, int lane) {
    const ftl_robot_params& p = (lane == 0) ? c.leader : (lane == 1 ? c.follower : c.bear);
    Limits L;
    L.min_speed = p.min_speed; L.max_speed = p.max_speed; L.max_rot = p.max_rotation_speed;
    L.max_dv = p.max_speed_change; L.max_drot = p.max_rotation_speed_change; L.img_w = p.img_w; L.img_h = p.img_h;
    return L;
}

__device__ __forceinline__ void command_turn(Robot& r, const Limits& L, double des, int dir) {
    r.des_rot_speed = (des <= L.max_rot) ? des : L.max_rot;
    r.des_rot_dir = dir;
}
__device__ __forceinline__ void command_forward(Robot& r, const Limits& L, double s) {
    if (s > L.max_speed) s = L.max_speed;
    if (s < L.min_speed) s = L.min_speed;
    r.des_speed = s;
}
__device__ __forceinline__ void robot_move(Robot& r, const Limits& L, bool active, double& dir_sin, double& dir_cos) {
    int rot_dir = r.rot_dir;
    if (rot_dir == 0) rot_dir = r.des_rot_dir;
    double change;
    if (rot_dir == r.des_rot_dir) {
        double needed = fabs(r.rot_speed - r.des_rot_speed);
        change = (needed <= L.max_drot) ? needed : L.max_drot;
        if (r.des_rot_speed < r.rot_speed) change = -1 * change;
    } else {
        double needed = fabs(r.des_rot_speed + r.rot_speed);
        change = -((needed <= L.max_drot) ? needed : L.max_drot);
    }
    double nr = r.rot_speed + change;
    if (nr < 0) rot_dir = -1 * rot_dir;
    double rot_speed = fabs(nr);
    double needed = fabs(r.speed - r.des_speed);
    double dv = (L.max_dv <= needed) ? L.max_dv : needed;
    if (r.speed > r.des_speed) dv = -1 * dv;
    double speed = r.speed + dv;

    double direction = r.direction;
    int rx = r.rx, ry = r.ry, rw = r.rw, rh = r.rh;
    bool turning = active && (rot_speed != 0);
    if (turning) direction = angle_correction(direction + rot_dir * rot_speed);
    double s, c;
    sincos_bounded(direction * kDeg2Rad, s, c);
    dir_sin = s; dir_cos = c;
    if (turning) {
        double a32 = (double)(float)(-direction);
        double vw = fabs(c) * L.img_w + fabs(s) * L.img_h, vh = fabs(s) * L.img_w + fabs(c) * L.img_h;
        double tol = (double)(L.img_w + L.img_h) * 1e-6;
        double fw = vw - floor(vw), fh = vh - floor(vh);
        bool exact = (rint(a32 * (1.0 / 90.0)) * 90.0 == a32) || fw < tol || fw > 1.0 - tol || fh < tol || fh > 1.0 - tol;
        int nw = (int)vw, nh = (int)vh;
        if (exact) rotate_size(L.img_w, L.img_h, -direction, nw, nh);
        int cx = rx + (rw >> 1), cy = ry + (rh >> 1);
        rw = nw; rh = nh; rx = cx - (nw >> 1); ry = cy - (nh >> 1);
    }
    float mx = (float)(c * speed), my = (float)(s * speed);
    float px = r.px + mx, py = r.py + my;
    double dx = (double)px - (double)(rx + (rw >> 1));
    double dy = (double)py - (double)(ry + (rh >> 1));
    rx += (int)dx; ry += (int)dy;
    if (active) {
        r.rot_dir = rot_dir; r.rot_speed = rot_speed; r.speed = speed; r.direction = direction;
        r.px = px; r.py = py; r.rx = rx; r.ry = ry; r.rw = rw; r.rh = rh;
    }
}
__device__ __forceinline__ int angle_to_point_int(double cx, double cy, double tx, double ty) {
#ifndef FTL_FAST_ATAN
    return (int)angle_to_point(cx, cy, tx, ty);
#else
    const double rx = tx - cx, ry = ty - cy;
    if (rx == 0.0) return 0;
    const float fx = (float)rx, fy = (float)ry;
    const float ax = fabsf(fx), ay = fabsf(fy);
    const float hi = fmaxf(ax, ay), lo = fminf(ax, ay);
    const float a = lo / hi;
    const float t = a * a;
    float p = __builtin_fmaf(t, -0.0117212f, 0.05265332f);
    p = __builtin_fmaf(t, p, -0.11643287f); p = __builtin_fmaf(t, p, 0.19354346f); p = __builtin_fmaf(t, p, -0.33262347f); p = __builtin_fmaf(t, p, 0.99997726f);
    float d = a * p * 57.29577951308232f;
    d = ay > ax ? 90.0f - d : d;
    d = fx < 0.0f ? 180.0f - d : d;
    d = fy < 0.0f ? 360.0f - d : d;
    const float fl = floorf(d), fr = d - fl;
    if (fr > 2.0e-3f && fr < 1.0f - 2.0e-3f) return (int)fl;
    return (int)angle_to_point(cx, cy, tx, ty);
#endif
}

__device__ __forceinline__ void steer_to_point(Robot& r, const Limits& L, double tx, double ty, bool has_speed, double speed) {
    double new_speed = has_speed ? speed : euclid_f64((double)r.px, (double)r.py, tx, ty);
    int desirable = angle_to_point_int((double)r.px, (double)r.py, tx, ty);
    int cur = (int)r.direction;
    int delta, dir;
    if (desirable - cur > 0) {
        if (desirable - cur > 180) { delta = cur + (360 - desirable); dir = -1; }
        else { delta = desirable - cur; dir = 1; }
    } else {
        if (cur - desirable > 180) { dir = 1; delta = (360 - cur) + desirable; }
        else { dir = -1; delta = cur - desirable; }
    }
    command_turn(r, L, (double)delta, dir);
    command_forward(r, L, new_speed);
}

__device__ __forceinline__ bool rects_collide(int ax, int ay, int aw, int ah, int bx, int by, int bw, int bh) {
    if (aw == 0 || ah == 0 || bw == 0 || bh == 0) return false;
    return ax < bx + bw && ay < by + bh && ax + aw > bx && ay + ah > by;
}

__device__ __forceinline__ double* hist_slot(const FtlDevParams& P, int env, int abs_idx) {
    return P.hist + ((size_t)env * P.cfg.corr_cap + (abs_idx & (P.cfg.corr_cap - 1))) * 2;
}
__device__ __forceinline__ double* corr_slot(const FtlDevParams& P, int env, int abs_idx) {
    return P.corr + ((size_t)env * P.cfg.corr_cap + (abs_idx & (P.cfg.corr_cap - 1))) * 4;
}
__device__ __forceinline__ float4* corr32_slot(const FtlDevParams& P, int env, int abs_idx) {
    return reinterpret_cast<float4*>(P.corr32) + (size_t)env * P.cfg.corr_cap + (abs_idx & (P.cfg.corr_cap - 1));
}
enum { SEG_STATIC = 0, SEG_DYNAMIC = 1, SEG_CORRIDOR = 2, SEG_GREEN = 3, SEG_CLASSES = 4 };

__device__ __forceinline__ bool hit_segment(float cx, float cy, double ex, double ey, float ex32, float ey32, float4 sg, double& d2) {
    const float ax = sg.x, ay = sg.y, bx = sg.z, by = sg.w;
    float cax = cx - ax, cay = cy - ay, cbx = cx - bx, cby = cy - by, bax = bx - ax, bay = by - ay;
    bool t3 = cay * bax > bay * cax;
    float fdax = ex32 - ax, fday = ey32 - ay, fdbx = ex32 - bx, fdby = ey32 - by;
    float s1 = fday * cax - cay * fdax, s2 = fdby * cbx - cby * fdbx, s4 = fday * bax - bay * fdax;
    bool t1 = s1 > 0.0f, t2 = s2 > 0.0f, t4 = s4 > 0.0f;
    if (!(fabsf(s1) > 0.5f && fabsf(s2) > 0.5f && fabsf(s4) > 0.5f)) {
        double day = ey - (double)ay, dax = ex - (double)ax, dby = ey - (double)by, dbx = ex - (double)bx;
        t1 = day * (double)cax > (double)cay * dax;
        t2 = dby * (double)cbx > (double)cby * dbx;
        t4 = day * (double)bax > (double)bay * dax;
    }
    if (!((t1 != t2) && (t3 != t4))) return false;
    double rbx = ex - (double)cx, rby = ey - (double)cy;
    float dpx = ax - cx, dpy = ay - cy;
    float dapx = -bay, dapy = bax;
    double denom = (double)dapx * rbx + (double)dapy * rby;
    float num = dapx * dpx + dapy * dpy;
    double t = (double)num / denom;
    double x = t * rbx + (double)cx, y = t * rby + (double)cy;
    double qx = x - (double)cx, qy = y - (double)cy;
    d2 = qx * qx + qy * qy;
    return true;
}

}

__device__ __forceinline__ float arc_atan2(float y, float x) {
    const float ax = fabsf(x), ay = fabsf(y);
    const float hi = fmaxf(ax, ay), lo = fminf(ax, ay);
    const float a = hi > 0.0f ? __fdividef(lo, hi) : 0.0f;
    const float t = a * a;
    float r = a * __builtin_fmaf(t, __builtin_fmaf(t, __builtin_fmaf(t, __builtin_fmaf(t, 0.0208351f, -0.0851330f), 0.1801410f), -0.3302995f), 0.9998660f);
    r = ay > ax ? 1.5707963267948966f - r : r;
    r = x < 0.0f ? 3.141592653589793f - r : r;
    return y < 0.0f ? -r : r;
}

#ifdef FTL_PROFILE_RAYS
__device__ unsigned long long g_rcyc[16];
__shared__ unsigned long long s_rcyc[16];
#define FTL_RTIC(slot) do { unsigned long long _t = __builtin_readcyclecounter(); if (threadIdx.x == 0) s_rcyc[slot] += _t - _rprev; _rprev = _t; } while (0)
#define FTL_RTIC_INIT unsigned long long _rprev = __builtin_readcyclecounter()
#else
#define FTL_RTIC(slot) do { } while (0)
#define FTL_RTIC_INIT do { } while (0)
#endif

#define FTL_FOR_LASERS(k) _Pragma("unroll") for (int k = 0; k < FTL_MAX_LASERS; k++) if (k < c.n_lasers && !(EXPL && c.lasers[k].compas))

template <int HM, bool EXPL = false, bool SPLIT = false, bool CAPPED = false>
__global__ void __launch_bounds__(FTL_WAVE, FTL_RAYS_WPE) ftl_rays_kernel(const FtlDevParams* __restrict__ Pp, const FtlCall C) {
    extern __shared__ __align__(16) unsigned char lds[];
    using namespace ftl;
    const FtlDevParams& P = *Pp;
    const ftl_config& c = P.cfg;
    int env = blockIdx.x;
    if (SPLIT) {
        const int gslot = ((int)(blockIdx.x / C.epw) * C.parts + C.part) * C.epw + (int)(blockIdx.x % C.epw);
        if (gslot >= P.n_envs) return;
        env = P.perm ? P.perm[gslot] : gslot;
    }
    if (env >= P.n_envs) return;
    if (C.mode == 1 && C.mask && !C.mask[env]) return;
    const int lane = threadIdx.x;
#ifdef FTL_PROFILE_RAYS
    if (lane < 16) s_rcyc[lane] = 0;
    __syncthreads();
#endif
    FTL_RTIC_INIT;
    const int hmax = P.hmax;
    const int nrect_dyn = P.R - 1;
    const int cmask = P.corr_lds_cap - 1;
    const int cap_rs = c.n_static + hmax, cap_rd = hmax * (P.R - 2 > 0 ? P.R - 2 : 0) + 1;
    const int cap_cr = 2 * P.corr_lds_cap, cap_gr = 2 * hmax;
    float4* s_corr = reinterpret_cast<float4*>(lds);
    int4* s_rect = reinterpret_cast<int4*>(s_corr + P.corr_lds_cap);
    float4* s_green = reinterpret_cast<float4*>(s_rect + cap_rs + cap_rd);
    unsigned* s_rmask = reinterpret_cast<unsigned*>(s_green + cap_gr);
    unsigned* s_cref = s_rmask + cap_rs + cap_rd;
    unsigned* s_gmask = s_cref + cap_cr;
    int* s_cnt = reinterpret_cast<int*>(s_gmask + cap_gr);
    int* s_ecnt = s_cnt + SEG_CLASSES;
    unsigned short* s_edge = reinterpret_cast<unsigned short*>(s_cnt + 8);
    const int n_u32 = (cap_rs + cap_rd) + cap_cr + cap_gr + 8 + 2 * (cap_rs + cap_rd);
    double2* s_ray = reinterpret_cast<double2*>(s_rmask + ((n_u32 + 3) & ~3));
    unsigned* s_best = reinterpret_cast<unsigned*>(s_ray + P.total_rays);
    float* s_miss = reinterpret_cast<float*>(s_best + (size_t)P.total_rays * HM);
    unsigned short* s_pair = reinterpret_cast<unsigned short*>(s_miss + P.total_rays);
    const unsigned kInfBits = 0x7f800000u;

    const int* ei = rec_field(P.env_int, P, env);
    const int* swp = rec_field(P.snap_win, P, env);
    const int4* srp = reinterpret_cast<const int4*>(rec_field(P.snap_rects, P, env));
    const int swv = lane < hmax * 4 ? swp[lane] : 0;
    const int eiv = lane < FTL_EI_COUNT ? ei[lane] : 0;
    const int fpv = lane < 2 ? __float_as_int(rec_field(P.rb_pos, P, env)[2 * 1 + lane]) : 0;
    const int fdv = lane < 2 ? reinterpret_cast<const int*>(rec_field(P.rb_dbl, P, env) + 1 * FTL_RD_COUNT + FTL_RD_DIRECTION)[lane] : 0;
    const int fcv = lane < 4 ? reinterpret_cast<const int*>(rec_field(P.fol_cs, P, env))[lane] : 0;
    const int scen = __builtin_amdgcn_readlane(eiv, FTL_EI_SCEN), snap_count = __builtin_amdgcn_readlane(eiv, FTL_EI_SNAP_COUNT);
    const int scan_ok = __builtin_amdgcn_readlane(eiv, FTL_EI_SCAN_OK), snap_head = __builtin_amdgcn_readlane(eiv, FTL_EI_SNAP_HEAD);
    const int newest = (snap_head == 0 ? hmax : snap_head) - 1;
    const float cx = __int_as_float(__builtin_amdgcn_readlane(fpv, 0)), cy = __int_as_float(__builtin_amdgcn_readlane(fpv, 1));
    const double fdir = __hiloint2double(__builtin_amdgcn_readlane(fdv, 1), __builtin_amdgcn_readlane(fdv, 0));
    const double fcd = __hiloint2double(__builtin_amdgcn_readlane(fcv, 1), __builtin_amdgcn_readlane(fcv, 0));
    const double fsd = __hiloint2double(__builtin_amdgcn_readlane(fcv, 3), __builtin_amdgcn_readlane(fcv, 2));
    float* out_base = C.out.lasers + (size_t)env * P.lasers_len;
    const int nsnap = snap_count < hmax ? snap_count : hmax;
    const unsigned all_snaps = (1u << nsnap) - 1u;
    const int4* stp = reinterpret_cast<const int4*>(P.scen.static_rects) + (size_t)scen * c.n_static;

#pragma nounroll
    for (int which = 0; which < 2; which++) {
        int lane_v = (int)threadIdx.x;
        asm volatile("" : "+v"(lane_v));
        const int lane = lane_v;
        const int n_rays = P.pass_rays[which], pbase = P.pass_base[which];
        if (n_rays == 0) continue;
        const float lmax = P.pass_lmax[which];
        const int ndyn = hmax * nrect_dyn;
        const bool merged = c.n_static + ndyn <= FTL_WAVE;
        const int dl = merged ? lane - c.n_static : lane;
        const int4 dynq = (dl >= 0 && dl < ndyn) ? srp[dl] : make_int4(0, 0, 0, 0);
        const int4 stq = lane < c.n_static ? stp[lane] : make_int4(0, 0, 0, 0);
        if (!((scan_ok >> which) & 1)) {
            for (int k = 0; k < c.n_lasers; k++) if (c.lasers[k].after_tracker == which && !(EXPL && c.lasers[k].compas)) {
                const int Wd = c.lasers[k].count * (c.lasers[k].pad_sectors ? 4 : 1);
                for (int i = lane; i < c.lasers[k].history * Wd; i += FTL_WAVE) {
                    out_base[c.lasers[k].out_offset + i] = (float)c.lasers[k].length;
                    if (C.out.policy_obs && P.pol_off[k] >= 0)
                        C.out.policy_obs[(size_t)env * P.pol_h * P.pol_width + (i / Wd) * P.pol_width + P.pol_off[k] + (i % Wd)] = 1.0f;
                }
            }
            continue;
        }
        int win_lo[HM], win_hi[HM];
        int umin = 0x7fffffff, umax = 0;
#pragma unroll
        for (int a = 0; a < HM; a++) {
            win_lo[a] = 0; win_hi[a] = 0;
            if (a < nsnap) {
                int slot = newest - a; slot += slot < 0 ? hmax : 0;
                win_lo[a] = __builtin_amdgcn_readlane(swv, 4 * slot + 2 * which); win_hi[a] = __builtin_amdgcn_readlane(swv, 4 * slot + 2 * which + 1);
                umin = min(umin, win_lo[a]); umax = max(umax, win_hi[a]);
            }
        }
        FTL_RTIC(7);
#if defined(FTL_RAYS_STOP) && FTL_RAYS_STOP == 0
        continue;
#endif
        __syncthreads();
        if (lane < SEG_CLASSES + 2) s_cnt[lane] = 0;
        const bool staged = !CAPPED || umax - umin <= P.corr_lds_cap;
        auto corr_f32 = [&](int p) { return *corr32_slot(P, env, p); };
        if (staged) for (int p = umin + lane; p < umax; p += FTL_WAVE) s_corr[p & cmask] = corr_f32(p);
        __syncthreads();
        FTL_RTIC(0);
#if defined(FTL_RAYS_STOP) && FTL_RAYS_STOP == 1
        continue;
#endif

        const float reach = lmax + 2.0f;
        const float bx0 = cx - reach, bx1 = cx + reach, by0 = cy - reach, by1 = cy + reach;
        auto push_rect = [&](int cls, int4 q, unsigned sm) {
            if (sm == 0u) return;
            const float l = (float)q.x, t = (float)q.y, r = (float)(q.x + q.z), b = (float)(q.y + q.w);
            if (r < bx0 || l > bx1 || b < by0 || t > by1) return;
            const int slot = (cls == SEG_STATIC ? 0 : cap_rs) + atomicAdd(&s_cnt[cls], 1);
            s_rect[slot] = q; s_rmask[slot] = sm;
            unsigned em = (cy > b ? 1u : 0u) | (cx > r ? 2u : 0u) | (cy < t ? 4u : 0u) | (cx < l ? 8u : 0u);
            if (em == 0u) em = 15u;
            int at = (cls == SEG_STATIC ? 0 : 4 * cap_rs) + atomicAdd(&s_ecnt[cls], __popc(em));
            while (em) { const int e = __ffs(em) - 1; em &= em - 1; s_edge[at++] = (unsigned short)((slot << 2) | e); }
        };
        auto push_corr = [&](int p, int side, float ax, float ay, float bx, float by, unsigned sm) {
            if (fmaxf(ax, bx) < bx0 || fminf(ax, bx) > bx1 || fmaxf(ay, by) < by0 || fminf(ay, by) > by1) return;
            s_cref[atomicAdd(&s_cnt[SEG_CORRIDOR], 1)] = (unsigned)(p & cmask) | ((unsigned)side << 15) | (sm << 16);
        };
        auto push_green = [&](float ax, float ay, float bx, float by, unsigned sm) {
            if (fmaxf(ax, bx) < bx0 || fminf(ax, bx) > bx1 || fmaxf(ay, by) < by0 || fminf(ay, by) > by1) return;
            int at = atomicAdd(&s_cnt[SEG_GREEN], 1);
            s_green[at] = make_float4(ax, ay, bx, by); s_gmask[at] = sm;
        };
        {
            const int dls = dl < 0 ? 0 : dl;
            const int slot = (int)(((unsigned)dls * P.inv_nrect_dyn) >> 16), o = dls - slot * nrect_dyn;
            int a = newest - slot; a += a < 0 ? hmax : 0;
            const unsigned sm_dyn = (dl >= 0 && dl < ndyn && a < nsnap) ? 1u << a : 0u;
            if (merged) {
                const bool is_st = lane < c.n_static;
                push_rect((is_st || o == 0) ? SEG_STATIC : SEG_DYNAMIC, is_st ? stq : dynq, is_st ? all_snaps : sm_dyn);
            } else {
                push_rect(SEG_STATIC, stq, lane < c.n_static ? all_snaps : 0u);
                for (int w = lane + FTL_WAVE; w < c.n_static; w += FTL_WAVE) push_rect(SEG_STATIC, stp[w], all_snaps);
                push_rect(o == 0 ? SEG_STATIC : SEG_DYNAMIC, dynq, sm_dyn);
            }
            if (staged) for (int p = umin + lane; p < umax - 1; p += FTL_WAVE) {
                unsigned sm = 0;
#pragma unroll
                for (int a = 0; a < HM; a++) if (a < nsnap && win_lo[a] <= p && p + 1 < win_hi[a]) sm |= 1u << a;
                if (sm) {
                    float4 u = s_corr[p & cmask], v = s_corr[(p + 1) & cmask];
                    push_corr(p, 0, u.x, u.y, v.x, v.y, sm);
                    push_corr(p, 1, u.z, u.w, v.z, v.w, sm);
                }
            }
            else if (lane == 0) s_cnt[SEG_CORRIDOR] = 2 * max(umax - umin - 1, 0);
            if (lane < nsnap) {
                int lo = 0, hi = 0;
#pragma unroll
                for (int j = 0; j < HM; j++) if (j == lane) { lo = win_lo[j]; hi = win_hi[j]; }
                float4 u = staged ? s_corr[lo & cmask] : corr_f32(lo), v = staged ? s_corr[(hi - 1) & cmask] : corr_f32(hi - 1);
                push_green(u.x, u.y, u.z, u.w, 1u << lane);
                push_green(v.x, v.y, v.z, v.w, 1u << lane);
            }
        }
        FTL_RTIC(1);
#if defined(FTL_RAYS_STOP) && FTL_RAYS_STOP == 2
        continue;
#endif
        {
            for (int g = lane; g < n_rays; g += FTL_WAVE) {
                const double2 rot = *reinterpret_cast<const double2*>(&P.ray_dir[pbase + g].c);
                const double len = P.ray_dir[pbase + g].len;
                const double co = fcd * rot.x - fsd * rot.y, s = fsd * rot.x + fcd * rot.y;
                const double ex = (double)cx + co * len, ey = (double)cy + s * len;
                s_ray[g] = make_double2(ex, ey);
                if (P.miss_const) s_miss[g] = (float)len;
                else { const double qx0 = ex - (double)cx, qy0 = ey - (double)cy; s_miss[g] = (float)sqrt(__builtin_fma(qy0, qy0, qx0 * qx0)); }
#pragma unroll
                for (int j = 0; j < HM; j++) s_best[j * P.total_rays + g] = kInfBits;
            }
        }
        __syncthreads();
        FTL_RTIC(2);
#if defined(FTL_RAYS_STOP) && FTL_RAYS_STOP == 3
        continue;
#endif

        {
            int cls_any = 0;
#pragma nounroll
            for (int k = 0; k < c.n_lasers; k++) { const unsigned fl = P.ray_sens[k].flags; if ((int)((fl >> 5) & 1u) == which && !(fl & 64u)) cls_any |= (int)(fl & 15u); }
            int cq[SEG_CLASSES];
#pragma unroll
            for (int q = 0; q < SEG_CLASSES; q++) cq[q] = ((cls_any >> q) & 1) ? (q < 2 ? s_ecnt[q] : s_cnt[q]) : 0;
            const int n_items = cq[0] + cq[1] + cq[2] + cq[3];
            auto fetch = [&](int mq, int m, float4& sg, unsigned& sm) {
                if (mq < 2) {
                    const int ent = s_edge[(mq == SEG_STATIC ? 0 : 4 * cap_rs) + m];
                    const int at = ent >> 2;
                    const int4 q = s_rect[at]; sm = s_rmask[at];
                    const float l = (float)q.x, t = (float)q.y, r = (float)(q.x + q.z), b = (float)(q.y + q.w);
                    const int e = ent & 3;
                    sg = e == 0 ? make_float4(l, b, r, b) : e == 1 ? make_float4(r, t, r, b) : e == 2 ? make_float4(r, t, l, t) : make_float4(l, b, l, t);
                } else if (mq == SEG_CORRIDOR) {
                    if (staged) {
                        const unsigned ref = s_cref[m];
                        const int p = ref & 0x7fff; sm = ref >> 16;
                        const float4 u = s_corr[p], v = s_corr[(p + 1) & cmask];
                        sg = (ref >> 15) & 1u ? make_float4(u.z, u.w, v.z, v.w) : make_float4(u.x, u.y, v.x, v.y);
                    } else {
                        const int p = umin + (m >> 1);
                        sm = 0;
#pragma unroll
                        for (int a = 0; a < HM; a++) if (a < nsnap && win_lo[a] <= p && p + 1 < win_hi[a]) sm |= 1u << a;
                        const float4 u = corr_f32(p), v = corr_f32(p + 1);
                        sg = (m & 1) ? make_float4(u.z, u.w, v.z, v.w) : make_float4(u.x, u.y, v.x, v.y);
                    }
                } else { sg = s_green[m]; sm = s_gmask[m]; }
            };
            auto test = [&](int ray, const float4& sgx, unsigned smx) {
                const double2 e = s_ray[ray];
                double d2;
                if (hit_segment(cx, cy, e.x, e.y, (float)e.x, (float)e.y, sgx, d2)) {
                    d2 = sqrt(d2);
                    const unsigned bits = __float_as_uint((float)d2);
#pragma unroll
                    for (int j = 0; j < HM; j++) if ((smx >> j) & 1u) atomicMin(&s_best[j * P.total_rays + ray], bits);
                }
            };
            const float fdir_rad = (float)(fdir * kDeg2Rad);
            int np_u = 0;
            for (int w0 = 0; w0 < n_items; w0 += FTL_WAVE) {
                const int w = w0 + lane;
                int m = -1, mq = 0;
                {
                    int j = 0, start = 0, end = 0;
#pragma unroll
                    for (int q = 0; q < SEG_CLASSES; q++) {
                        end += cq[q];
                        const bool past = w >= end;
                        j += past ? 1 : 0; start = past ? end : start;
                    }
                    if (w < n_items) { m = w - start; mq = j; }
                }
                FTL_RTIC(3);
                float4 sg = make_float4(0.f, 0.f, 0.f, 0.f); unsigned sm = 0;
                float a0 = 0.0f, wd = 0.0f, dmin2 = 3.0e38f;
                if (m >= 0) {
                    fetch(mq, m, sg, sm);
                    if (sm == 0u) m = -1;
                }
                if (m >= 0) {
                    const float ax = sg.x - cx, ay = sg.y - cy, bx = sg.z - cx, by = sg.w - cy;
                    const float angA = arc_atan2(ay, ax), angB = arc_atan2(by, bx);
                    float diff = angB - angA; if (diff < 0.0f) diff += 6.283185307179586f;
                    a0 = angA; wd = diff;
                    if (diff > 3.141592653589793f) { a0 = angB; wd = 6.283185307179586f - diff; }
                    a0 -= fdir_rad;
                    const float ex_ = bx - ax, ey_ = by - ay;
                    const float l2 = __builtin_fmaf(ex_, ex_, ey_ * ey_);
                    const float tt = l2 > 0.0f ? fminf(fmaxf(__fdividef(-__builtin_fmaf(ax, ex_, ay * ey_), l2), 0.0f), 1.0f) : 0.0f;
                    const float nx = __builtin_fmaf(tt, ex_, ax), ny = __builtin_fmaf(tt, ey_, ay);
                    dmin2 = __builtin_fmaf(nx, nx, ny * ny);
                }
                FTL_RTIC(4);
                auto flush = [&](int np) {
                    __syncthreads();
                    for (int p0 = 0; p0 < np; p0 += FTL_WAVE) {
                        const int p = p0 + lane;
                        const unsigned rec = p < np ? s_pair[p] : 0u;
                        const int L = (int)(rec >> 10);
                        const float4 sgp = make_float4(__shfl(sg.x, L), __shfl(sg.y, L), __shfl(sg.z, L), __shfl(sg.w, L));
                        const unsigned smp = (unsigned)__shfl((int)sm, L);
                        if (p < np) test((int)(rec & 1023u), sgp, smp);
                    }
                    __syncthreads();
                };
#pragma nounroll
                for (int k = 0; k < c.n_lasers; k++) {
                    const FtlRaySensor rs = P.ray_sens[k];
                    if ((int)((rs.flags >> 5) & 1u) != which || (rs.flags & 64u)) continue;
                    const int N = rs.count, rbase = rs.rbase;
                    int i0 = 0, cnt = 0;
                    if (m >= 0 && ((rs.flags >> mq) & 1u) && !(dmin2 > rs.reach2)) {
                        const float fN = (float)N;
                        const float wu = wd * rs.inv_step;
                        if ((rs.flags & 16u) || dmin2 < 4.0f || wu > 0.5f * fN - 0.05f) { i0 = 0; cnt = N; }
                        else {
                            float st = __builtin_fmaf(a0, rs.inv_step, -rs.off_u);
                            st = __builtin_fmaf(-floorf(st * rs.inv_count), fN, st);
                            i0 = (int)ceilf(st - rs.slack);
                            cnt = (int)floorf(st + wu + rs.slack) - i0 + 1;
                            cnt = cnt > N ? N : cnt;
                        }
                    }
#if defined(FTL_RAYS_STOP) && FTL_RAYS_STOP == 5
                    cnt = cnt == 0x7fffffff ? 1 : 0;
#endif
#ifdef FTL_PROFILE_RAYS
                    if (threadIdx.x == 0) { s_rcyc[8] += 1; }
                    { int mc = cnt; for (int o = 32; o >= 1; o >>= 1) mc = max(mc, __shfl_xor(mc, o)); int ni = __popcll(__ballot(m >= 0)); int sc = cnt; for (int o = 32; o >= 1; o >>= 1) sc += __shfl_xor(sc, o); if (threadIdx.x == 0) { s_rcyc[9] += mc; s_rcyc[10] += sc; s_rcyc[11] += ni; s_rcyc[12] += (mc <= 2); s_rcyc[13] += (mc > 2 && mc <= 4); s_rcyc[14] += (mc > 4 && mc <= 8); s_rcyc[15] += (mc > 8); } }
#endif
                    unsigned long long wide = __ballot(cnt > FTL_WIDE_ARC);
                    while (wide) {
                        const int L = __ffsll((long long)wide) - 1; wide &= wide - 1;
                        const int i0L = __builtin_amdgcn_readlane(i0, L), cntL = __builtin_amdgcn_readlane(cnt, L);
                        if (cntL > FTL_WAVE) {
                            const float4 sgL = make_float4(__int_as_float(__builtin_amdgcn_readlane(__float_as_int(sg.x), L)), __int_as_float(__builtin_amdgcn_readlane(__float_as_int(sg.y), L)),
                                                           __int_as_float(__builtin_amdgcn_readlane(__float_as_int(sg.z), L)), __int_as_float(__builtin_amdgcn_readlane(__float_as_int(sg.w), L)));
                            const unsigned smL = (unsigned)__builtin_amdgcn_readlane((int)sm, L);
                            for (int t = lane; t < cntL; t += FTL_WAVE) {
                                int i = i0L + t; i = i < 0 ? i + N : (i >= N ? i - N : i);
                                test(rbase + i, sgL, smL);
                            }
                            continue;
                        }
                        if (np_u + cntL > FTL_PAIR_CAP) { flush(np_u); np_u = 0; }
                        if (lane < cntL) {
                            int i = i0L + lane; i = i < 0 ? i + N : (i >= N ? i - N : i);
                            s_pair[np_u + lane] = (unsigned short)((L << 10) | (rbase + i));
                        }
                        np_u += cntL;
                    }
                    const int own = cnt > FTL_WIDE_ARC ? 0 : cnt;
                    int pre = 0, tot = 0;
#pragma unroll
                    for (int b = 0; b < 4; b++) if ((FTL_WIDE_ARC >> b) != 0) {
                        const unsigned long long bm = __ballot((own >> b) & 1);
                        pre += (int)__builtin_amdgcn_mbcnt_hi((unsigned)(bm >> 32), __builtin_amdgcn_mbcnt_lo((unsigned)bm, 0u)) << b;
                        tot += __popcll(bm) << b;
                    }
                    if (np_u + tot > FTL_PAIR_CAP) { flush(np_u); np_u = 0; }
                    for (int t = 0; t < own; t++) {
                        int i = i0 + t; i = i < 0 ? i + N : (i >= N ? i - N : i);
                        s_pair[np_u + pre + t] = (unsigned short)((lane << 10) | (rbase + i));
                    }
                    np_u += tot;
                }
                if (np_u > 0) { flush(np_u); np_u = 0; }
            }
        }
        FTL_RTIC(5);
#if defined(FTL_RAYS_STOP) && FTL_RAYS_STOP == 4
        continue;
#endif
        __syncthreads();
        {
            float* pol = C.out.policy_obs ? C.out.policy_obs + (size_t)env * P.pol_h * P.pol_width : nullptr;
            bool any_pad = false;
            FTL_FOR_LASERS(k) if (EXPL && c.lasers[k].after_tracker == which && c.lasers[k].pad_sectors) {
                any_pad = true;
                const int tot = c.lasers[k].history * 4 * c.lasers[k].count;
                for (int i = lane; i < tot; i += FTL_WAVE) out_base[c.lasers[k].out_offset + i] = 0.0f;
                if (pol && P.pol_off[k] >= 0) for (int i = lane; i < tot; i += FTL_WAVE) {
                    int row = i / (4 * c.lasers[k].count), col = i - row * 4 * c.lasers[k].count;
                    pol[row * P.pol_width + P.pol_off[k] + col] = 0.0f;
                }
            }
            if (any_pad) __syncthreads();
            if constexpr (!EXPL) {
                for (int g = lane; g < n_rays; g += FTL_WAVE) {
                    int i = g, H = 0, N = 0, ooff = 0, poff = -1; float flen = 1.0f; bool found = false;
                    FTL_FOR_LASERS(k) if (c.lasers[k].after_tracker == which) {
                        const int Nk = c.lasers[k].count;
                        if (!found && i < Nk) {
                            found = true; N = Nk; H = c.lasers[k].history; ooff = c.lasers[k].out_offset; poff = P.pol_off[k];
                            flen = (float)c.lasers[k].length;
                        }
                        if (!found) i -= Nk;
                    }
                    const float miss = s_miss[g];
#pragma unroll
                    for (int a2 = 0; a2 < HM; a2++) if (a2 < H) {
                        const unsigned bb = s_best[a2 * P.total_rays + g];
                        const float vf = (a2 < nsnap && bb != kInfBits) ? __uint_as_float(bb) : miss;
                        out_base[ooff + (H - 1 - a2) * N + i] = vf;
                        if (pol && poff >= 0) pol[(H - 1 - a2) * P.pol_width + poff + i] = fminf(fmaxf(vf / flen, 0.0f), 1.0f);
                    }
                }
            } else {
                int rbase = 0;
                FTL_FOR_LASERS(k) {
                    const int N = c.lasers[k].count;
                    if (c.lasers[k].after_tracker != which) { continue; }
                    const int H = c.lasers[k].history, ooff = c.lasers[k].out_offset, poff = P.pol_off[k], rb = rbase;
                    const bool pad = c.lasers[k].pad_sectors != 0;
                    const float flen = (float)c.lasers[k].length;
                    const int Wd = pad ? 4 * N : N;
                    for (int q = lane; q < N * H; q += FTL_WAVE) {
                        int a2 = 0;
#pragma unroll
                        for (int j = 1; j < HM; j++) a2 += (q >= j * N) ? 1 : 0;
                        const int i = q - a2 * N;
                        int col = i;
                        if (pad) {
                            const double lis = (double)N / 4.0, di = (double)i;
                            col = (di < lis ? 0 : (di < 2 * lis ? 1 : (di < 3 * lis ? 2 : 3))) * N + i;
                        }
                        const unsigned bb = s_best[a2 * P.total_rays + rb + i];
                        const float vf = (a2 < nsnap && bb != kInfBits) ? __uint_as_float(bb) : s_miss[rb + i];
                        out_base[ooff + (H - 1 - a2) * Wd + col] = vf;
                        if (pol && poff >= 0) pol[(H - 1 - a2) * P.pol_width + poff + col] = fminf(fmaxf(vf / flen, 0.0f), 1.0f);
                    }
                    rbase += N;
                }
            }
        }
        FTL_RTIC(6);
    }
#ifdef FTL_PROFILE_RAYS
    __syncthreads();
    if (lane < 16) atomicAdd(&g_rcyc[lane], s_rcyc[lane]);
#endif
}
```

Baseline: 268.2 million.

## Precompute ray-kernel LDS layout on host and reload params per pass

Result: no change. 269.1 million, median of 5 (+0.3%).

```diff
diff --git a/continiousenvironment_follower_leader_amd/_lib.py b/continiousenvironment_follower_leader_amd/_lib.py
--- a/continiousenvironment_follower_leader_amd/_lib.py
+++ b/continiousenvironment_follower_leader_amd/_lib.py
@@ -106,6 +106,8 @@
     lib.ftl_sampler_refresh.restype = C.c_int
     lib.ftl_sampler_start.argtypes = [vp, C.POINTER(abi.Outputs), vp]
     lib.ftl_sampler_start.restype = C.c_int
+    lib.ftl_debug_ray_layout.argtypes = [vp, C.POINTER(i32), i32]
+    lib.ftl_debug_ray_layout.restype = C.c_int
     lib.ftl_gz_create.argtypes = [vp, i32, i32, C.POINTER(vp)]
     lib.ftl_gz_destroy.argtypes = [vp]
     lib.ftl_gz_destroy.restype = None
diff --git a/continiousenvironment_follower_leader_amd/abi.py b/continiousenvironment_follower_leader_amd/abi.py
--- a/continiousenvironment_follower_leader_amd/abi.py
+++ b/continiousenvironment_follower_leader_amd/abi.py
@@ -206,3 +206,22 @@
 class RenderParams(C.Structure):
     _fields_ = [("width", C.c_int32), ("height", C.c_int32), ("scale", C.c_float), ("origin_x", C.c_float), ("origin_y", C.c_float),
                 ("layers", C.c_uint32), ("_pad", C.c_int32)]
+
+
+FTL_HMAX = 12
+RAY_LAYOUT_FIELDS = ("off_corr", "off_rect", "off_green", "off_rmask", "off_cref", "off_gmask", "off_cnt", "off_edge",
+                     "off_ray", "off_best", "off_miss", "off_pair", "lds_bytes", "best_rows", "cap_rs", "cap_rd",
+                     "cap_rs4", "cmask", "ndyn", "merged", "inv_nrect_dyn", "total_rays", "hmax", "nrect_dyn",
+                     "corr_lds_cap", "n_static", "_pad0", "_pad1") + tuple("best_row%d" % j for j in range(FTL_HMAX))
+RAY_PAIR_CAP = 192
+
+
+def ray_layout(lib, h):
+    buf = (C.c_int32 * len(RAY_LAYOUT_FIELDS))()
+    rc = lib.ftl_debug_ray_layout(h, buf, len(RAY_LAYOUT_FIELDS))
+    if rc != 0:
+        raise RuntimeError(lib.ftl_last_error().decode("utf-8", "replace"))
+    d = dict(zip(RAY_LAYOUT_FIELDS, list(buf)))
+    d["best_row"] = [d.pop("best_row%d" % j) for j in range(FTL_HMAX)]
+    d["inv_nrect_dyn"] &= 0xffffffff
+    return d
diff --git a/continiousenvironment_follower_leader_amd/csrc/ftl_abi.hip b/continiousenvironment_follower_leader_amd/csrc/ftl_abi.hip
--- a/continiousenvironment_follower_leader_amd/csrc/ftl_abi.hip
+++ b/continiousenvironment_follower_leader_amd/csrc/ftl_abi.hip
@@ -50,6 +50,7 @@
     int rg_slots, rg_epw;
     hipStream_t side; hipEvent_t ev_fork, ev_join; bool split;
     int win_base, win_count, win_stride;
+    size_t lds_pad_rays;
     size_t lds_pad;
     float* last_lasers;
     FtlQueueState* queue;
@@ -223,7 +224,6 @@
                      | (l.explicit_angles ? 16u : 0u) | (which ? 32u : 0u) | (l.compas ? 64u : 0u);
             if (!l.compas) rb[which] += l.count;
         }
-        P.inv_nrect_dyn = (65536u + (unsigned)(P.R - 1) - 1u) / (unsigned)(P.R - 1);
         int g = 0;
         for (int which = 0; which < 2; which++) {
             P.pass_base[which] = g; P.pass_lmax[which] = 0.0f;
@@ -284,10 +284,31 @@
         const size_t rects = (size_t)cfg->n_static + hmax + (size_t)hmax * (P.R - 2 > 0 ? P.R - 2 : 0) + 1;
         P.corr_lds_cap = cfg->corr_cap < 128 ? cfg->corr_cap : 128;
         if (const char* lc = getenv("FTL_DEBUG_CORR_LDS_CAP")) { int v = atoi(lc); if (v >= 2 && v <= cfg->corr_cap && (v & (v - 1)) == 0) P.corr_lds_cap = v; }
-        P.lds_rays = (int)((size_t)P.corr_lds_cap * 16 + rects * 20 + (size_t)2 * P.corr_lds_cap * 4 + (size_t)2 * hmax * 20 + 64
-                           + (size_t)rays * 16 + (size_t)rays * (hmax <= 5 ? 5 : FTL_HMAX) * 4       + (size_t)rays * 4
-                           + rects * 8 + 32
-                           + (size_t)FTL_PAIR_CAP * 2 + 16);
+        FtlRayLayout& L = P.lay;
+        L.hmax = hmax; L.nrect_dyn = P.R - 1; L.n_static = cfg->n_static; L.total_rays = rays; L.corr_lds_cap = P.corr_lds_cap;
+        L.cap_rs = cfg->n_static + hmax; L.cap_rd = hmax * (P.R - 2 > 0 ? P.R - 2 : 0) + 1;
+        L.cap_rs4 = 4 * L.cap_rs; L.cmask = P.corr_lds_cap - 1;
+        L.ndyn = hmax * (P.R - 1); L.merged = cfg->n_static + L.ndyn <= FTL_WAVE ? 1 : 0;
+        L.inv_nrect_dyn = (65536u + (unsigned)(P.R - 1) - 1u) / (unsigned)(P.R - 1);
+        L.best_rows = hmax <= 5 ? 5 : FTL_HMAX;
+        const size_t cap_gr = (size_t)2 * hmax, cap_cr = (size_t)2 * P.corr_lds_cap;
+        size_t o = 0;
+        auto place = [&o](size_t bytes, size_t align) { o = align_up(o, align); const size_t at = o; o += bytes; return (int32_t)at; };
+        L.off_corr = place((size_t)P.corr_lds_cap * 16, 16);
+        L.off_rect = place(rects * 16, 16);
+        L.off_green = place(cap_gr * 16, 16);
+        L.off_rmask = place(rects * 4, 4);
+        L.off_cref = place(cap_cr * 4, 4);
+        L.off_gmask = place(cap_gr * 4, 4);
+        L.off_cnt = place(8 * 4, 4);
+        L.off_edge = place(rects * 4 * 2, 2);
+        L.off_ray = place((size_t)rays * 16, 16);
+        L.off_best = place((size_t)rays * L.best_rows * 4, 4);
+        L.off_miss = place((size_t)rays * 4, 4);
+        L.off_pair = place((size_t)FTL_PAIR_CAP * 2, 2);
+        for (int j = 0; j < FTL_HMAX; j++) L.best_row[j] = L.off_best + 4 * (j < L.best_rows ? j : 0) * rays;
+        if (o > (size_t)64 * 1024) { delete h; return fail(FTL_E_INVALID, "config needs more than 64 KiB of LDS per env"); }
+        L.lds_bytes = (int32_t)o;
     }
     {
         const int f_max = cfg->rand_fps_hi > 0 ? cfg->rand_fps_hi - 1 : cfg->frames_per_step;
@@ -297,10 +318,10 @@
         if (set_lanes(h)) { delete h; return fail(FTL_E_INVALID, "the frame kernel needs more than 64 KiB of LDS per wavefront (static rects x frames per step)"); }
     }
     auto debug_pad = [](const char* name) { const char* v = getenv(name); const int p = v ? atoi(v) : 0; return p < 0 ? 0 : (p > 48 * 1024 ? 48 * 1024 : p); };
-    P.lds_rays += debug_pad("FTL_DEBUG_LDS_PAD_RAYS");
+    h->lds_pad_rays = (size_t)debug_pad("FTL_DEBUG_LDS_PAD_RAYS");
     h->lds_pad = (size_t)debug_pad("FTL_DEBUG_LDS_PAD");
-    if (getenv("FTL_DEBUG_PRINT_LDS")) fprintf(stderr, "ftl: ray kernel LDS %d B per env\n", P.lds_rays);
-    if (P.lds_rays > 64 * 1024) { delete h; return fail(FTL_E_INVALID, "config needs more than 64 KiB of LDS per env"); }
+    if (getenv("FTL_DEBUG_PRINT_LDS")) fprintf(stderr, "ftl: ray kernel LDS %d B per env\n", (int)(P.lay.lds_bytes + h->lds_pad_rays));
+    if (P.lay.lds_bytes + h->lds_pad_rays > 64 * 1024) { delete h; return fail(FTL_E_INVALID, "config needs more than 64 KiB of LDS per env"); }
     if (ftl_aux_lds_bytes(*cfg) > 64 * 1024) { delete h; return fail(FTL_E_INVALID, "the compas / lidar / radar sensors of this config need more than 64 KiB of LDS per env"); }
     *out = h;
     return FTL_OK;
@@ -479,9 +500,10 @@
             for (int k = 0; k < h->P.cfg.n_lasers; k++) expl = expl || h->P.cfg.lasers[k].explicit_angles != 0 || h->P.cfg.lasers[k].pad_sectors != 0 || h->P.cfg.lasers[k].compas != 0;
             const dim3 rgrid(count);
 #define FTL_LAUNCH_RAYS(HM_, EXPL_, SPLIT_) do { \
-                if (capped) hipLaunchKernelGGL((ftl_rays_kernel<HM_, EXPL_, SPLIT_, true>), rgrid, block, h->P.lds_rays, s, h->dP, c2); \
-                else hipLaunchKernelGGL((ftl_rays_kernel<HM_, EXPL_, SPLIT_, false>), rgrid, block, h->P.lds_rays, s, h->dP, c2); } while (0)
+                if (capped) hipLaunchKernelGGL((ftl_rays_kernel<HM_, EXPL_, SPLIT_, true>), rgrid, block, rays_lds, s, h->dP, c2); \
+                else hipLaunchKernelGGL((ftl_rays_kernel<HM_, EXPL_, SPLIT_, false>), rgrid, block, rays_lds, s, h->dP, c2); } while (0)
             const bool capped = h->P.corr_lds_cap < h->P.cfg.corr_cap;
+            const size_t rays_lds = (size_t)h->P.lay.lds_bytes + h->lds_pad_rays;
             if (parts > 1) {
                 if (!expl && h->P.hmax > 5 && h->P.hmax <= 10) FTL_LAUNCH_RAYS(10, false, true);
                 else if (h->P.hmax <= 5) FTL_LAUNCH_RAYS(5, true, true);
@@ -658,6 +680,12 @@
 #include "ftl_queue.hpp"
 #include "ftl_sampler.hpp"
 
+extern "C" int ftl_debug_ray_layout(const ftl_handle* h, int32_t* out, int n) {
+    if (!h || !out || n != (int)(sizeof(FtlRayLayout) / 4)) return fail(FTL_E_INVALID, "ftl_debug_ray_layout: null argument or a size other than the record's");
+    memcpy(out, &h->P.lay, sizeof(FtlRayLayout));
+    return FTL_OK;
+}
+
 #ifdef FTL_WAVE_TIMES
 extern "C" int ftl_debug_wave_timeline(unsigned long long* times, unsigned int* info) {
     hipDeviceSynchronize();
diff --git a/continiousenvironment_follower_leader_amd/csrc/ftl_device.hpp b/continiousenvironment_follower_leader_amd/csrc/ftl_device.hpp
--- a/continiousenvironment_follower_leader_amd/csrc/ftl_device.hpp
+++ b/continiousenvironment_follower_leader_amd/csrc/ftl_device.hpp
@@ -25,9 +25,19 @@
     uint32_t flags;
 };
 struct alignas(16) FtlRayDir { double c, s, len, _pad; };
+struct alignas(32) FtlRayLayout {
+    int32_t off_corr, off_rect, off_green, off_rmask, off_cref, off_gmask, off_cnt, off_edge;
+    int32_t off_ray, off_best, off_miss, off_pair, lds_bytes, best_rows, cap_rs, cap_rd;
+    int32_t cap_rs4, cmask, ndyn, merged;
+    uint32_t inv_nrect_dyn;
+    int32_t total_rays, hmax, nrect_dyn;
+    int32_t corr_lds_cap, n_static, _pad[2];
+    int32_t best_row[FTL_HMAX];
+};
+static_assert(sizeof(FtlRayLayout) == 160, "FtlRayLayout: ftl_debug_ray_layout hands it out as 40 int32");
 struct FtlDevParams {
     ftl_config cfg;
-    int32_t n_envs, R, lasers_len, total_rays, hmax, lds_rays;
+    int32_t n_envs, R, lasers_len, total_rays, hmax, _pad_hmax;
     int32_t pass_rays[2], pass_base[2];
     float pass_lmax[2];
     int32_t _pad_pass[2];
@@ -42,13 +52,14 @@
     float* corr32;
     float* hist1;
     double* fol_cs;
+    FtlRayLayout lay;
     FtlRayDir ray_dir[FTL_MAX_RAYS];
     FtlRaySensor ray_sens[FTL_MAX_LASERS];
-    uint32_t inv_nrect_dyn;
-    int32_t miss_const;
+    int32_t _pad_miss, miss_const;
     int32_t* perm; uint8_t* keys; uint16_t* rank; int32_t* bh;
     ftl_scenarios scen;
 };
+static_assert(offsetof(FtlDevParams, lay) % 32 == 0 && offsetof(FtlDevParams, ray_dir) == offsetof(FtlDevParams, lay) + sizeof(FtlRayLayout), "lay: one 32-byte aligned block, so that a scalar load of eight of its words never straddles a cache line");
 static_assert(sizeof(FtlRayDir) == 32 && offsetof(FtlDevParams, ray_dir) % 32 == 0, "ray_dir: 16-byte loads of its records must be aligned, and a record must not straddle a cache line (the device copy is 256-byte aligned)");
 struct FtlCall {
     const double* action; const int32_t* scen_idx; const uint8_t* mask;
@@ -334,7 +345,14 @@
 #define FTL_RTIC_INIT do { } while (0)
 #endif
 
+__device__ __forceinline__ const FtlDevParams* ray_params(const FtlDevParams* __restrict__ Pp) {
+    unsigned z;
+    asm volatile("s_mov_b32 %0, 0" : "=s"(z));
+    return reinterpret_cast<const FtlDevParams*>(reinterpret_cast<const char*>(Pp) + z);
+}
+
 #define FTL_FOR_LASERS(k) _Pragma("unroll") for (int k = 0; k < FTL_MAX_LASERS; k++) if (k < c.n_lasers && !(EXPL && c.lasers[k].compas))
+#define FTL_LDS_AT(T, off) reinterpret_cast<T*>(lds + (off))
 
 template <int HM, bool EXPL = false, bool SPLIT = false, bool CAPPED = false>
 __global__ void __launch_bounds__(FTL_WAVE, FTL_RAYS_WPE) ftl_rays_kernel(const FtlDevParams* __restrict__ Pp, const FtlCall C) {
@@ -346,7 +364,7 @@
     if (SPLIT) {
         const int gslot = ((int)(blockIdx.x / C.epw) * C.parts + C.part) * C.epw + (int)(blockIdx.x % C.epw);
         if (gslot >= P.n_envs) return;
-        env = P.perm ? P.perm[gslot] : gslot;
+        env = __builtin_amdgcn_readfirstlane(P.perm ? P.perm[gslot] : gslot);
     }
     if (env >= P.n_envs) return;
     if (C.mode == 1 && C.mask && !C.mask[env]) return;
@@ -356,30 +374,11 @@
     __syncthreads();
 #endif
     FTL_RTIC_INIT;
+    const unsigned kInfBits = 0x7f800000u;
     const int hmax = P.hmax;
-    const int nrect_dyn = P.R - 1;
-    const int cmask = P.corr_lds_cap - 1;
-    const int cap_rs = c.n_static + hmax, cap_rd = hmax * (P.R - 2 > 0 ? P.R - 2 : 0) + 1;
-    const int cap_cr = 2 * P.corr_lds_cap, cap_gr = 2 * hmax;
-    float4* s_corr = reinterpret_cast<float4*>(lds);
-    int4* s_rect = reinterpret_cast<int4*>(s_corr + P.corr_lds_cap);
-    float4* s_green = reinterpret_cast<float4*>(s_rect + cap_rs + cap_rd);
-    unsigned* s_rmask = reinterpret_cast<unsigned*>(s_green + cap_gr);
-    unsigned* s_cref = s_rmask + cap_rs + cap_rd;
-    unsigned* s_gmask = s_cref + cap_cr;
-    int* s_cnt = reinterpret_cast<int*>(s_gmask + cap_gr);
-    int* s_ecnt = s_cnt + SEG_CLASSES;
-    unsigned short* s_edge = reinterpret_cast<unsigned short*>(s_cnt + 8);
-    const int n_u32 = (cap_rs + cap_rd) + cap_cr + cap_gr + 8 + 2 * (cap_rs + cap_rd);
-    double2* s_ray = reinterpret_cast<double2*>(s_rmask + ((n_u32 + 3) & ~3));
-    unsigned* s_best = reinterpret_cast<unsigned*>(s_ray + P.total_rays);
-    float* s_miss = reinterpret_cast<float*>(s_best + (size_t)P.total_rays * HM);
-    unsigned short* s_pair = reinterpret_cast<unsigned short*>(s_miss + P.total_rays);
-    const unsigned kInfBits = 0x7f800000u;
 
     const int* ei = rec_field(P.env_int, P, env);
     const int* swp = rec_field(P.snap_win, P, env);
-    const int4* srp = reinterpret_cast<const int4*>(rec_field(P.snap_rects, P, env));
     const int swv = lane < hmax * 4 ? swp[lane] : 0;
     const int eiv = lane < FTL_EI_COUNT ? ei[lane] : 0;
     const int fpv = lane < 2 ? __float_as_int(rec_field(P.rb_pos, P, env)[2 * 1 + lane]) : 0;
@@ -387,30 +386,36 @@
     const int fcv = lane < 4 ? reinterpret_cast<const int*>(rec_field(P.fol_cs, P, env))[lane] : 0;
     const int scen = __builtin_amdgcn_readlane(eiv, FTL_EI_SCEN), snap_count = __builtin_amdgcn_readlane(eiv, FTL_EI_SNAP_COUNT);
     const int scan_ok = __builtin_amdgcn_readlane(eiv, FTL_EI_SCAN_OK), snap_head = __builtin_amdgcn_readlane(eiv, FTL_EI_SNAP_HEAD);
-    const int newest = (snap_head == 0 ? hmax : snap_head) - 1;
+    const int newest_e = (snap_head == 0 ? hmax : snap_head) - 1;
     const float cx = __int_as_float(__builtin_amdgcn_readlane(fpv, 0)), cy = __int_as_float(__builtin_amdgcn_readlane(fpv, 1));
     const double fdir = __hiloint2double(__builtin_amdgcn_readlane(fdv, 1), __builtin_amdgcn_readlane(fdv, 0));
+    const float fdir_rad = __int_as_float(__builtin_amdgcn_readfirstlane(__float_as_int((float)(fdir * kDeg2Rad))));
     const double fcd = __hiloint2double(__builtin_amdgcn_readlane(fcv, 1), __builtin_amdgcn_readlane(fcv, 0));
     const double fsd = __hiloint2double(__builtin_amdgcn_readlane(fcv, 3), __builtin_amdgcn_readlane(fcv, 2));
-    float* out_base = C.out.lasers + (size_t)env * P.lasers_len;
-    const int nsnap = snap_count < hmax ? snap_count : hmax;
-    const unsigned all_snaps = (1u << nsnap) - 1u;
-    const int4* stp = reinterpret_cast<const int4*>(P.scen.static_rects) + (size_t)scen * c.n_static;
+    const int nsnap_e = snap_count < hmax ? snap_count : hmax;
 
 #pragma nounroll
     for (int which = 0; which < 2; which++) {
         int lane_v = (int)threadIdx.x;
         asm volatile("" : "+v"(lane_v));
         const int lane = lane_v;
-        const int n_rays = P.pass_rays[which], pbase = P.pass_base[which];
-        if (n_rays == 0) continue;
+        int nsnap = nsnap_e, newest = newest_e;
+        asm volatile("" : "+s"(nsnap), "+s"(newest));
+        const FtlDevParams& P = *ray_params(Pp);
+        const ftl_config& c = P.cfg;
+        const FtlRayLayout& L = P.lay;
+        if (P.pass_rays[which] == 0) continue;
         const float lmax = P.pass_lmax[which];
-        const int ndyn = hmax * nrect_dyn;
-        const bool merged = c.n_static + ndyn <= FTL_WAVE;
-        const int dl = merged ? lane - c.n_static : lane;
+        const int hmax = L.hmax, nrect_dyn = L.nrect_dyn, cmask = L.cmask;
+        const int ndyn = L.ndyn, n_static = L.n_static;
+        const bool merged = L.merged != 0;
+        const int4* srp = reinterpret_cast<const int4*>(rec_field(P.snap_rects, P, env));
+        const int4* stp = reinterpret_cast<const int4*>(P.scen.static_rects) + (size_t)scen * n_static;
+        const int dl = merged ? lane - n_static : lane;
         const int4 dynq = (dl >= 0 && dl < ndyn) ? srp[dl] : make_int4(0, 0, 0, 0);
-        const int4 stq = lane < c.n_static ? stp[lane] : make_int4(0, 0, 0, 0);
+        const int4 stq = lane < n_static ? stp[lane] : make_int4(0, 0, 0, 0);
         if (!((scan_ok >> which) & 1)) {
+            float* out_base = C.out.lasers + (size_t)env * P.lasers_len;
             for (int k = 0; k < c.n_lasers; k++) if (c.lasers[k].after_tracker == which && !(EXPL && c.lasers[k].compas)) {
                 const int Wd = c.lasers[k].count * (c.lasers[k].pad_sectors ? 4 : 1);
                 for (int i = lane; i < c.lasers[k].history * Wd; i += FTL_WAVE) {
@@ -437,49 +442,54 @@
         continue;
 #endif
         __syncthreads();
-        if (lane < SEG_CLASSES + 2) s_cnt[lane] = 0;
-        const bool staged = !CAPPED || umax - umin <= P.corr_lds_cap;
-        auto corr_f32 = [&](int p) { return *corr32_slot(P, env, p); };
-        if (staged) for (int p = umin + lane; p < umax; p += FTL_WAVE) s_corr[p & cmask] = corr_f32(p);
+        if (lane < SEG_CLASSES + 2) FTL_LDS_AT(int, L.off_cnt)[lane] = 0;
+        const bool staged = !CAPPED || umax - umin <= L.corr_lds_cap;
+        auto corr_f32 = [&](const FtlDevParams& Pq, int p) { return *corr32_slot(Pq, env, p); };
+        if (staged) for (int p = umin + lane; p < umax; p += FTL_WAVE) FTL_LDS_AT(float4, L.off_corr)[p & cmask] = corr_f32(P, p);
         __syncthreads();
         FTL_RTIC(0);
 #if defined(FTL_RAYS_STOP) && FTL_RAYS_STOP == 1
         continue;
 #endif
 
+        const unsigned all_snaps = (1u << nsnap) - 1u;
+        const float4* s_corr = FTL_LDS_AT(float4, L.off_corr);
+        int* s_cnt = FTL_LDS_AT(int, L.off_cnt);
+        int* s_ecnt = s_cnt + SEG_CLASSES;
         const float reach = lmax + 2.0f;
         const float bx0 = cx - reach, bx1 = cx + reach, by0 = cy - reach, by1 = cy + reach;
         auto push_rect = [&](int cls, int4 q, unsigned sm) {
             if (sm == 0u) return;
             const float l = (float)q.x, t = (float)q.y, r = (float)(q.x + q.z), b = (float)(q.y + q.w);
             if (r < bx0 || l > bx1 || b < by0 || t > by1) return;
-            const int slot = (cls == SEG_STATIC ? 0 : cap_rs) + atomicAdd(&s_cnt[cls], 1);
-            s_rect[slot] = q; s_rmask[slot] = sm;
+            const int slot = (cls == SEG_STATIC ? 0 : L.cap_rs) + atomicAdd(&s_cnt[cls], 1);
+            FTL_LDS_AT(int4, L.off_rect)[slot] = q; FTL_LDS_AT(unsigned, L.off_rmask)[slot] = sm;
             unsigned em = (cy > b ? 1u : 0u) | (cx > r ? 2u : 0u) | (cy < t ? 4u : 0u) | (cx < l ? 8u : 0u);
             if (em == 0u) em = 15u;
-            int at = (cls == SEG_STATIC ? 0 : 4 * cap_rs) + atomicAdd(&s_ecnt[cls], __popc(em));
+            int at = (cls == SEG_STATIC ? 0 : L.cap_rs4) + atomicAdd(&s_ecnt[cls], __popc(em));
+            unsigned short* s_edge = FTL_LDS_AT(unsigned short, L.off_edge);
             while (em) { const int e = __ffs(em) - 1; em &= em - 1; s_edge[at++] = (unsigned short)((slot << 2) | e); }
         };
         auto push_corr = [&](int p, int side, float ax, float ay, float bx, float by, unsigned sm) {
             if (fmaxf(ax, bx) < bx0 || fminf(ax, bx) > bx1 || fmaxf(ay, by) < by0 || fminf(ay, by) > by1) return;
-            s_cref[atomicAdd(&s_cnt[SEG_CORRIDOR], 1)] = (unsigned)(p & cmask) | ((unsigned)side << 15) | (sm << 16);
+            FTL_LDS_AT(unsigned, L.off_cref)[atomicAdd(&s_cnt[SEG_CORRIDOR], 1)] = (unsigned)(p & cmask) | ((unsigned)side << 15) | (sm << 16);
         };
         auto push_green = [&](float ax, float ay, float bx, float by, unsigned sm) {
             if (fmaxf(ax, bx) < bx0 || fminf(ax, bx) > bx1 || fmaxf(ay, by) < by0 || fminf(ay, by) > by1) return;
             int at = atomicAdd(&s_cnt[SEG_GREEN], 1);
-            s_green[at] = make_float4(ax, ay, bx, by); s_gmask[at] = sm;
+            FTL_LDS_AT(float4, L.off_green)[at] = make_float4(ax, ay, bx, by); FTL_LDS_AT(unsigned, L.off_gmask)[at] = sm;
         };
         {
             const int dls = dl < 0 ? 0 : dl;
-            const int slot = (int)(((unsigned)dls * P.inv_nrect_dyn) >> 16), o = dls - slot * nrect_dyn;
+            const int slot = (int)(((unsigned)dls * L.inv_nrect_dyn) >> 16), o = dls - slot * nrect_dyn;
             int a = newest - slot; a += a < 0 ? hmax : 0;
             const unsigned sm_dyn = (dl >= 0 && dl < ndyn && a < nsnap) ? 1u << a : 0u;
             if (merged) {
-                const bool is_st = lane < c.n_static;
+                const bool is_st = lane < n_static;
                 push_rect((is_st || o == 0) ? SEG_STATIC : SEG_DYNAMIC, is_st ? stq : dynq, is_st ? all_snaps : sm_dyn);
             } else {
-                push_rect(SEG_STATIC, stq, lane < c.n_static ? all_snaps : 0u);
-                for (int w = lane + FTL_WAVE; w < c.n_static; w += FTL_WAVE) push_rect(SEG_STATIC, stp[w], all_snaps);
+                push_rect(SEG_STATIC, stq, lane < n_static ? all_snaps : 0u);
+                for (int w = lane + FTL_WAVE; w < n_static; w += FTL_WAVE) push_rect(SEG_STATIC, stp[w], all_snaps);
                 push_rect(o == 0 ? SEG_STATIC : SEG_DYNAMIC, dynq, sm_dyn);
             }
             if (staged) for (int p = umin + lane; p < umax - 1; p += FTL_WAVE) {
@@ -497,7 +507,7 @@
                 int lo = 0, hi = 0;
 #pragma unroll
                 for (int j = 0; j < HM; j++) if (j == lane) { lo = win_lo[j]; hi = win_hi[j]; }
-                float4 u = staged ? s_corr[lo & cmask] : corr_f32(lo), v = staged ? s_corr[(hi - 1) & cmask] : corr_f32(hi - 1);
+                float4 u = staged ? s_corr[lo & cmask] : corr_f32(P, lo), v = staged ? s_corr[(hi - 1) & cmask] : corr_f32(P, hi - 1);
                 push_green(u.x, u.y, u.z, u.w, 1u << lane);
                 push_green(v.x, v.y, v.z, v.w, 1u << lane);
             }
@@ -507,16 +517,20 @@
         continue;
 #endif
         {
+            const FtlDevParams& P = *ray_params(Pp);
+            const FtlRayLayout& L = P.lay;
+            const int n_rays = P.pass_rays[which], pbase = P.pass_base[which];
             for (int g = lane; g < n_rays; g += FTL_WAVE) {
                 const double2 rot = *reinterpret_cast<const double2*>(&P.ray_dir[pbase + g].c);
                 const double len = P.ray_dir[pbase + g].len;
                 const double co = fcd * rot.x - fsd * rot.y, s = fsd * rot.x + fcd * rot.y;
                 const double ex = (double)cx + co * len, ey = (double)cy + s * len;
-                s_ray[g] = make_double2(ex, ey);
+                float* s_miss = FTL_LDS_AT(float, L.off_miss);
+                FTL_LDS_AT(double2, L.off_ray)[g] = make_double2(ex, ey);
                 if (P.miss_const) s_miss[g] = (float)len;
                 else { const double qx0 = ex - (double)cx, qy0 = ey - (double)cy; s_miss[g] = (float)sqrt(__builtin_fma(qy0, qy0, qx0 * qx0)); }
 #pragma unroll
-                for (int j = 0; j < HM; j++) s_best[j * P.total_rays + g] = kInfBits;
+                for (int j = 0; j < HM; j++) FTL_LDS_AT(unsigned, L.best_row[j])[g] = kInfBits;
             }
         }
         __syncthreads();
@@ -526,24 +540,29 @@
 #endif
 
         {
+            const FtlDevParams& P = *ray_params(Pp);
+            const ftl_config& c = P.cfg;
+            const FtlRayLayout& L = P.lay;
+            const int cmask = L.cmask;
+            const float4* s_corr = FTL_LDS_AT(float4, L.off_corr);
             int cls_any = 0;
 #pragma nounroll
             for (int k = 0; k < c.n_lasers; k++) { const unsigned fl = P.ray_sens[k].flags; if ((int)((fl >> 5) & 1u) == which && !(fl & 64u)) cls_any |= (int)(fl & 15u); }
             int cq[SEG_CLASSES];
 #pragma unroll
-            for (int q = 0; q < SEG_CLASSES; q++) cq[q] = ((cls_any >> q) & 1) ? (q < 2 ? s_ecnt[q] : s_cnt[q]) : 0;
+            for (int q = 0; q < SEG_CLASSES; q++) cq[q] = ((cls_any >> q) & 1) ? FTL_LDS_AT(int, L.off_cnt)[q < 2 ? SEG_CLASSES + q : q] : 0;
             const int n_items = cq[0] + cq[1] + cq[2] + cq[3];
             auto fetch = [&](int mq, int m, float4& sg, unsigned& sm) {
                 if (mq < 2) {
-                    const int ent = s_edge[(mq == SEG_STATIC ? 0 : 4 * cap_rs) + m];
+                    const int ent = FTL_LDS_AT(unsigned short, L.off_edge)[(mq == SEG_STATIC ? 0 : L.cap_rs4) + m];
                     const int at = ent >> 2;
-                    const int4 q = s_rect[at]; sm = s_rmask[at];
+                    const int4 q = FTL_LDS_AT(int4, L.off_rect)[at]; sm = FTL_LDS_AT(unsigned, L.off_rmask)[at];
                     const float l = (float)q.x, t = (float)q.y, r = (float)(q.x + q.z), b = (float)(q.y + q.w);
                     const int e = ent & 3;
                     sg = e == 0 ? make_float4(l, b, r, b) : e == 1 ? make_float4(r, t, r, b) : e == 2 ? make_float4(r, t, l, t) : make_float4(l, b, l, t);
                 } else if (mq == SEG_CORRIDOR) {
                     if (staged) {
-                        const unsigned ref = s_cref[m];
+                        const unsigned ref = FTL_LDS_AT(unsigned, L.off_cref)[m];
                         const int p = ref & 0x7fff; sm = ref >> 16;
                         const float4 u = s_corr[p], v = s_corr[(p + 1) & cmask];
                         sg = (ref >> 15) & 1u ? make_float4(u.z, u.w, v.z, v.w) : make_float4(u.x, u.y, v.x, v.y);
@@ -552,22 +571,21 @@
                         sm = 0;
 #pragma unroll
                         for (int a = 0; a < HM; a++) if (a < nsnap && win_lo[a] <= p && p + 1 < win_hi[a]) sm |= 1u << a;
-                        const float4 u = corr_f32(p), v = corr_f32(p + 1);
+                        const float4 u = corr_f32(P, p), v = corr_f32(P, p + 1);
                         sg = (m & 1) ? make_float4(u.z, u.w, v.z, v.w) : make_float4(u.x, u.y, v.x, v.y);
                     }
-                } else { sg = s_green[m]; sm = s_gmask[m]; }
+                } else { sg = FTL_LDS_AT(float4, L.off_green)[m]; sm = FTL_LDS_AT(unsigned, L.off_gmask)[m]; }
             };
             auto test = [&](int ray, const float4& sgx, unsigned smx) {
-                const double2 e = s_ray[ray];
+                const double2 e = FTL_LDS_AT(double2, L.off_ray)[ray];
                 double d2;
                 if (hit_segment(cx, cy, e.x, e.y, (float)e.x, (float)e.y, sgx, d2)) {
                     d2 = sqrt(d2);
                     const unsigned bits = __float_as_uint((float)d2);
 #pragma unroll
-                    for (int j = 0; j < HM; j++) if ((smx >> j) & 1u) atomicMin(&s_best[j * P.total_rays + ray], bits);
+                    for (int j = 0; j < HM; j++) if ((smx >> j) & 1u) atomicMin(&FTL_LDS_AT(unsigned, L.best_row[j])[ray], bits);
                 }
             };
-            const float fdir_rad = (float)(fdir * kDeg2Rad);
             int np_u = 0;
             for (int w0 = 0; w0 < n_items; w0 += FTL_WAVE) {
                 const int w = w0 + lane;
@@ -607,10 +625,10 @@
                     __syncthreads();
                     for (int p0 = 0; p0 < np; p0 += FTL_WAVE) {
                         const int p = p0 + lane;
-                        const unsigned rec = p < np ? s_pair[p] : 0u;
-                        const int L = (int)(rec >> 10);
-                        const float4 sgp = make_float4(__shfl(sg.x, L), __shfl(sg.y, L), __shfl(sg.z, L), __shfl(sg.w, L));
-                        const unsigned smp = (unsigned)__shfl((int)sm, L);
+                        const unsigned rec = p < np ? FTL_LDS_AT(unsigned short, L.off_pair)[p] : 0u;
+                        const int Ls = (int)(rec >> 10);
+                        const float4 sgp = make_float4(__shfl(sg.x, Ls), __shfl(sg.y, Ls), __shfl(sg.z, Ls), __shfl(sg.w, Ls));
+                        const unsigned smp = (unsigned)__shfl((int)sm, Ls);
                         if (p < np) test((int)(rec & 1023u), sgp, smp);
                     }
                     __syncthreads();
@@ -642,12 +660,12 @@
 #endif
                     unsigned long long wide = __ballot(cnt > FTL_WIDE_ARC);
                     while (wide) {
-                        const int L = __ffsll((long long)wide) - 1; wide &= wide - 1;
-                        const int i0L = __builtin_amdgcn_readlane(i0, L), cntL = __builtin_amdgcn_readlane(cnt, L);
+                        const int Lw = __ffsll((long long)wide) - 1; wide &= wide - 1;
+                        const int i0L = __builtin_amdgcn_readlane(i0, Lw), cntL = __builtin_amdgcn_readlane(cnt, Lw);
                         if (cntL > FTL_WAVE) {
-                            const float4 sgL = make_float4(__int_as_float(__builtin_amdgcn_readlane(__float_as_int(sg.x), L)), __int_as_float(__builtin_amdgcn_readlane(__float_as_int(sg.y), L)),
-                                                           __int_as_float(__builtin_amdgcn_readlane(__float_as_int(sg.z), L)), __int_as_float(__builtin_amdgcn_readlane(__float_as_int(sg.w), L)));
-                            const unsigned smL = (unsigned)__builtin_amdgcn_readlane((int)sm, L);
+                            const float4 sgL = make_float4(__int_as_float(__builtin_amdgcn_readlane(__float_as_int(sg.x), Lw)), __int_as_float(__builtin_amdgcn_readlane(__float_as_int(sg.y), Lw)),
+                                                           __int_as_float(__builtin_amdgcn_readlane(__float_as_int(sg.z), Lw)), __int_as_float(__builtin_amdgcn_readlane(__float_as_int(sg.w), Lw)));
+                            const unsigned smL = (unsigned)__builtin_amdgcn_readlane((int)sm, Lw);
                             for (int t = lane; t < cntL; t += FTL_WAVE) {
                                 int i = i0L + t; i = i < 0 ? i + N : (i >= N ? i - N : i);
                                 test(rbase + i, sgL, smL);
@@ -657,7 +675,7 @@
                         if (np_u + cntL > FTL_PAIR_CAP) { flush(np_u); np_u = 0; }
                         if (lane < cntL) {
                             int i = i0L + lane; i = i < 0 ? i + N : (i >= N ? i - N : i);
-                            s_pair[np_u + lane] = (unsigned short)((L << 10) | (rbase + i));
+                            FTL_LDS_AT(unsigned short, L.off_pair)[np_u + lane] = (unsigned short)((Lw << 10) | (rbase + i));
                         }
                         np_u += cntL;
                     }
@@ -672,7 +690,7 @@
                     if (np_u + tot > FTL_PAIR_CAP) { flush(np_u); np_u = 0; }
                     for (int t = 0; t < own; t++) {
                         int i = i0 + t; i = i < 0 ? i + N : (i >= N ? i - N : i);
-                        s_pair[np_u + pre + t] = (unsigned short)((lane << 10) | (rbase + i));
+                        FTL_LDS_AT(unsigned short, L.off_pair)[np_u + pre + t] = (unsigned short)((lane << 10) | (rbase + i));
                     }
                     np_u += tot;
                 }
@@ -685,6 +703,12 @@
 #endif
         __syncthreads();
         {
+            const FtlDevParams& P = *ray_params(Pp);
+            const ftl_config& c = P.cfg;
+            const FtlRayLayout& L = P.lay;
+            const int n_rays = P.pass_rays[which];
+            float* out_base = C.out.lasers + (size_t)env * P.lasers_len;
+            const float* s_miss = FTL_LDS_AT(float, L.off_miss);
             float* pol = C.out.policy_obs ? C.out.policy_obs + (size_t)env * P.pol_h * P.pol_width : nullptr;
             bool any_pad = false;
             FTL_FOR_LASERS(k) if (EXPL && c.lasers[k].after_tracker == which && c.lasers[k].pad_sectors) {
@@ -711,7 +735,7 @@
                     const float miss = s_miss[g];
 #pragma unroll
                     for (int a2 = 0; a2 < HM; a2++) if (a2 < H) {
-                        const unsigned bb = s_best[a2 * P.total_rays + g];
+                        const unsigned bb = FTL_LDS_AT(unsigned, L.best_row[a2])[g];
                         const float vf = (a2 < nsnap && bb != kInfBits) ? __uint_as_float(bb) : miss;
                         out_base[ooff + (H - 1 - a2) * N + i] = vf;
                         if (pol && poff >= 0) pol[(H - 1 - a2) * P.pol_width + poff + i] = fminf(fmaxf(vf / flen, 0.0f), 1.0f);
@@ -736,7 +760,7 @@
                             const double lis = (double)N / 4.0, di = (double)i;
                             col = (di < lis ? 0 : (di < 2 * lis ? 1 : (di < 3 * lis ? 2 : 3))) * N + i;
                         }
-                        const unsigned bb = s_best[a2 * P.total_rays + rb + i];
+                        const unsigned bb = FTL_LDS_AT(unsigned, L.off_best)[a2 * L.total_rays + rb + i];
                         const float vf = (a2 < nsnap && bb != kInfBits) ? __uint_as_float(bb) : s_miss[rb + i];
                         out_base[ooff + (H - 1 - a2) * Wd + col] = vf;
                         if (pol && poff >= 0) pol[(H - 1 - a2) * P.pol_width + poff + col] = fminf(fmaxf(vf / flen, 0.0f), 1.0f);
```
